# dsshim0125/s2p

Measured on AMD Instinct MI355X. Metric: G+D train-step images/sec at 84x84 bs=64/GPU, higher is better.
Workload: dtype bf16; 1 GPU; configs[2]: full G+D train step (hinge GAN + feature matching + VGG19 perceptual + L1, Adam x2), 84x84 cheetah, netG=s2p, netD=multiscale(2); global_batch=64, per_gpu_batch=64, parallelism=dp1, hip_graph=True, graph_segments=1, streams=overlapped, vgg_weights=seeded stand-in (ImageNet weights unobtainable offline)

## Files before the change

### include/s2p_hip.h

```cpp
#ifndef S2P_HIP_H
#define S2P_HIP_H
#include <stddef.h>
#include <stdint.h>

#ifdef __cplusplus
extern "C" {
#endif
#pragma GCC visibility push(default)

#define S2P_VERSION 125

enum { S2P_F32 = 0, S2P_BF16 = 1 };
enum { S2P_ACT_NONE = 0, S2P_ACT_RELU = 1, S2P_ACT_LRELU = 2, S2P_ACT_TANH = 3, S2P_ACT_SWISH = 4 };
enum { S2P_EPI_STORE = 0,
       S2P_EPI_ADD = 1,
       S2P_EPI_MUL_ACTGRAD = 2   };

typedef struct {
  int32_t dtype;
  int32_t N, H, W, Cin, x_pitch;
  int32_t Ho, Wo, Cout, y_pitch;
  int32_t KH, KW, stride, pad;
  int32_t transposed;
  int32_t reflect;
  int32_t groups;
  int32_t x_gstride, y_gstride;
  int32_t cin_real;
} s2p_conv_desc;

int s2p_version(void);
const char* s2p_last_error(void);

int s2p_conv2d_fwd(const s2p_conv_desc* d, const void* x, const void* w_fwd, const float* bias,
                   const void* aux, void* y, int act, float slope, int epi, void* stream);
int s2p_conv2d_dgrad(const s2p_conv_desc* d, const void* dy, const void* w_bwd,
                     const void* aux, const void* aux2, void* dx, int epi, int aux_act, float slope,
                     void* stream);
size_t s2p_conv2d_fwd_workspace(const s2p_conv_desc* d, int epi);
int s2p_conv2d_fwd_ws(const s2p_conv_desc* d, const void* x, const void* w_fwd, const float* bias,
                      const void* aux, void* y, int act, float slope, int epi, void* workspace,
                      size_t workspace_bytes, void* stream);
size_t s2p_conv2d_dgrad_workspace(const s2p_conv_desc* d);
int s2p_conv2d_dgrad_ws(const s2p_conv_desc* d, const void* dy, const void* w_bwd,
                        const void* aux, const void* aux2, void* dx, int epi, int aux_act, float slope,
                        void* workspace, size_t workspace_bytes, void* stream);
int s2p_conv2d_fwd_mat(const s2p_conv_desc* d, const void* x, const void* w_fwd, const float* bias, const void* aux,
                       void* y, int epi, const void* gb_img, int gb_pitch, const float* gb_st, int gb_st_pitch,
                       int act, float slope, float eps, void* y_mat, int y_mat_pitch, float* stats, void* workspace,
                       size_t workspace_bytes, void* stream);
int s2p_conv2d_dgrad_mat(const s2p_conv_desc* d, const void* dy, const void* w_bwd, void* d_mid, const void* aux, const void* xn,
                         int xn_pitch, const float* stats, const void* gb_img, int gb_pitch, const float* gb_st,
                         int gb_st_pitch, int act, float slope, float eps, float* sums, void* dxn, int dxn_pitch,
                         void* dgb_img, int dgb_pitch, float* dgb_st, int dgb_st_pitch, const void* res, int res_pitch,
                         void* workspace, size_t workspace_bytes, void* stream);
int s2p_conv2d_mat_is_fused(const s2p_conv_desc* d, int dgrad, int has_gb);
int s2p_conv2d_wgrad(const s2p_conv_desc* d, const void* x, const void* dy, float* dw, float* db,
                     int cin_real, int cout_real, int64_t dw_gstride, int splitk, void* stream);
size_t s2p_conv2d_wgrad_workspace(const s2p_conv_desc* d, int cin_real, int cout_real);
int s2p_conv2d_wgrad_ws(const s2p_conv_desc* d, const void* x, const void* dy, float* dw, float* db,
                        int cin_real, int cout_real, int64_t dw_gstride, int splitk, void* workspace,
                        size_t workspace_bytes, void* stream);
size_t s2p_conv2d_wgrad_det_workspace(const s2p_conv_desc* d, int cin_real, int cout_real, int splitk);
typedef struct { const void* x; const void* dy; float* dw; float* db; } s2p_wgrad_job;
size_t s2p_conv2d_wgrad_batched_workspace(const s2p_conv_desc* d, int n_jobs, int cin_real, int cout_real);
int s2p_conv2d_wgrad_batched(const s2p_conv_desc* d, const s2p_wgrad_job* jobs, int n_jobs, int cin_real,
                             int cout_real, void* workspace, size_t workspace_bytes, void* stream);
int s2p_reflect_pad_bwd(int dtype, const void* dxp, int N, int H, int W, int C, int pad, void* dx,
                        void* stream);
int s2p_channel_sum(int dtype, const void* dy, int64_t pixels, int C, int pitch, float* db,
                    void* stream);
size_t s2p_channel_sum_workspace(int64_t pixels, int C);
int s2p_channel_sum_ws(int dtype, const void* dy, int64_t pixels, int C, int pitch, float* db, void* workspace,
                       size_t workspace_bytes, void* stream);

int64_t s2p_in_stats_floats(int N, int HW, int C);
int s2p_in_stats(int dtype, const void* x, int N, int HW, int C, int pitch, float eps,
                 float* stats, void* stream);
int s2p_in_apply_fwd(int dtype, const void* x, int N, int HW, int C, int pitch,
                     const float* stats, const void* gb_img, int gb_pitch,
                     const float* gb_st, int gb_st_pitch, int act, float slope, float eps,
                     void* y, int y_pitch, void* stream);
int s2p_in_norm_fwd(int dtype, const void* x, int N, int HW, int C, int pitch, const void* gb_img, int gb_pitch,
                    const float* gb_st, int gb_st_pitch, int act, float slope, float eps, void* y, int y_pitch,
                    float* stats, void* stream);
int64_t s2p_in_bwd_sums_floats(int N, int HW, int C);
int s2p_in_bwd_reduce(int dtype, const void* da, int da_pitch, const void* x, int N, int HW, int C,
                      int pitch, const float* stats, const void* gb_img, int gb_pitch,
                      const float* gb_st, int gb_st_pitch, int act, float slope, float eps,
                      float* sums, void* stream);
int s2p_in_bwd_apply(int dtype, const void* da, int da_pitch, const void* x, int N, int HW, int C,
                     int pitch, const float* stats, const void* gb_img, int gb_pitch,
                     const float* gb_st, int gb_st_pitch, int act, float slope, float eps,
                     const float* sums, void* dx, int dx_pitch, void* dgb_img, int dgb_pitch,
                     float* dgb_st, int dgb_st_pitch, void* stream);

int s2p_posenc_fwd(const float* state, int N, int S, int L, float* out, int out_pitch, void* stream);

int s2p_in_norm_bwd(int dtype, const void* da, int da_pitch, const void* x, int N, int HW, int C, int pitch,
                    const float* stats, const void* gb_img, int gb_pitch, const float* gb_st, int gb_st_pitch,
                    int act, float slope, float eps, float* sums, void* dx, int dx_pitch, void* dgb_img,
                    int dgb_pitch, float* dgb_st, int dgb_st_pitch, void* stream);
int s2p_in_norm_bwd_res(int dtype, const void* da, int da_pitch, const void* x, int N, int HW, int C, int pitch,
                        const float* stats, const void* gb_img, int gb_pitch, const float* gb_st, int gb_st_pitch,
                        int act, float slope, float eps, float* sums, void* dx, int dx_pitch, void* dgb_img,
                        int dgb_pitch, float* dgb_st, int dgb_st_pitch, const void* res, int res_pitch, void* stream);

int s2p_linear_fwd(const float* x, int M, int K, int x_pitch, const float* w, int w_row, const float* bias, int N,
                   int act, float slope, float* y, int y_pitch, int n_store, void* stream);
size_t s2p_linear_bwd_workspace(int M, int K, int N);
int s2p_linear_bwd(const float* x, int x_pitch, const float* dy, int dy_pitch, const float* y, int y_pitch, int M,
                   int K, int k_real, int N, const float* w_bwd, int wb_row, int act, float slope, float* dw,
                   int dw_row, float* db, float* dx, int dx_pitch, void* workspace, size_t workspace_bytes,
                   void* stream);

int s2p_gauss_head_fwd(const float* raw, int raw_pitch, int M, int D, const float* eps, int eps_pitch, float* mean,
                       int mean_pitch, float* std, int std_pitch, float* z, int z_pitch, float* z2, int z2_pitch,
                       void* stream);
int s2p_gauss_head_bwd(const float* raw, int raw_pitch, int M, int D, const float* eps, int eps_pitch, const float* dmean,
                       int dmean_pitch, const float* dstd, int dstd_pitch, const float* dz, int dz_pitch, const float* dz2,
                       int dz2_pitch, float* draw, int draw_pitch, void* stream);
int s2p_linear_add_fwd(const float* x, int M, int K, int x_pitch, const float* w, int w_row, const float* bias, int N,
                       const float* add, int add_pitch, int act, float slope, float* y, int y_pitch, int n_store,
                       void* stream);
int s2p_linear_add_bwd(const float* x, int x_pitch, const float* dy, int dy_pitch, const float* y, int y_pitch, int M,
                       int K, int k_real, int N, const float* w_bwd, int wb_row, int act, float slope, float* dw,
                       int dw_row, float* db, float* dx, int dx_pitch, int dx_accumulate, float* dadd, int dadd_pitch,
                       void* stream);
int s2p_gauss_kl(const float* mu_p, const float* std_p, int p_pitch, const float* mu_q, const float* std_q, int q_pitch,
                 int B, int T, int D, int const_first, float scale, float* loss, float* dmu_p, float* dstd_p,
                 int dp_pitch, float* dmu_q, float* dstd_q, int dq_pitch, void* stream);
int s2p_gauss_ll(const float* mu, int mu_pitch, const float* std, int std_pitch, const float* target, const float* done,
                 int64_t n, float scale, float* loss, float* dmu, float* dstd, void* stream);
int s2p_gauss_ll_image(int dtype, const void* mu, int pitch, const void* target, int target_u8, int N, int C, int HW,
                       float sigma, float scale, float* loss, void* dmu, void* stream);

int s2p_avgpool3x3s2_fwd(int dtype, const void* x, int N, int H, int W, int C, void* y, void* stream);
int s2p_avgpool3x3s2_bwd(int dtype, const void* dy, int N, int H, int W, int C, void* dx,
                         int accumulate, void* stream);
int s2p_maxpool2x2_fwd(int dtype, const void* x, int N, int H, int W, int C, void* y, void* stream);
int s2p_maxpool2x2_bwd(int dtype, const void* dy, const void* x, int N, int H, int W, int C,
                       void* dx, void* stream);
int s2p_resize_nearest(int dtype, const void* x, int N, int H, int W, int C, void* y, int Ho, int Wo,
                       void* stream);
int s2p_nchw_to_nhwc(int dtype, const float* x, int N, int C, int H, int W, void* y, int y_pitch,
                     int c_off, int zero_pad, void* stream);
int s2p_nhwc_to_nchw(int dtype, const void* x, int x_pitch, int c_off, int N, int C, int H, int W,
                     float* y, int accumulate, void* stream);
int s2p_u8_to_nhwc(int dtype, const void* x, int64_t pixels, int C, void* y, int y_pitch, void* stream);
int s2p_nhwc_to_u8(int dtype, const void* x, int x_pitch, int64_t pixels, int C, void* y, void* stream);
int s2p_cast(int src_dtype, const void* src, int dst_dtype, void* dst, int64_t n, void* stream);

int s2p_l1_loss(int dtype, const void* a, const void* b, int64_t count, float scale,
                float* loss_out, void* grad_a, int accumulate, void* stream);
#define S2P_L1_MAX_JOBS 16
typedef struct { const void* a; const void* b; void* grad_a; int64_t count; float scale; float* loss_out; } s2p_l1_job;
int s2p_l1_loss_multi(int dtype, const s2p_l1_job* jobs, int n_jobs, void* stream);
int s2p_hinge_loss(int dtype, const void* x, int64_t count, int mode, float scale,
                   float* loss_out, void* grad_x, void* stream);
int s2p_hinge_loss_strided(int dtype, const void* x, int64_t pixels, int pitch, int mode, float scale,
                           float* loss_out, void* grad_x, void* stream);

int s2p_ensemble_head(const float* raw, int raw_pitch, const float* xin, int x_pitch, int B, int E, int D,
                      const float* min_logstd, const float* max_logstd, float* mean, float* std,
                      const int32_t* pick, const float* obs_mean, const float* obs_std, float rew_mean,
                      float rew_std, float* next_obs, float* reward, float* disagreement, float* aleatoric,
                      void* stream);

int s2p_ensemble_linear_fwd(const float* x, int64_t x_gstride, int x_pitch, const float* w, const float* bias,
                            const int32_t* member, int G, int E, int B, int K, int N, float* pre, float* act, int y_pitch,
                            void* stream);
int s2p_ensemble_linear_bwd(const float* x, int64_t x_gstride, int x_pitch, const float* dpre, int dpre_pitch,
                            const float* w, const int32_t* member, int G, int E, int B, int K, int N, float* dw, float* db,
                            const float* pre_prev, float* dprev, int prev_pitch, void* stream);
int s2p_ensemble_nll(const float* raw, int raw_pitch, const float* xin, int64_t x_gstride, int x_pitch, const float* target,
                     int64_t t_gstride, int t_pitch, int B, int G, int D, const float* min_logstd, const float* max_logstd,
                     float scale, float bound_reg, float* sums, float* loss, float* draw, int draw_pitch, float* dmin_logstd,
                     float* dmax_logstd, float* mean, float* std, void* stream);

int s2p_adam_step(float* p, const float* g, float* m, float* v, int64_t n, float lr, float beta1,
                  float beta2, float eps, int step, float grad_scale, void* stream);
int s2p_adam_step_dev(float* p, const float* g, float* m, float* v, int64_t n, float lr, float beta1,
                      float beta2, float eps, int* step_dev, float grad_scale, void* stream);
int s2p_adam_step_dev_part(float* p, const float* g, float* m, float* v, int64_t n, float lr, float beta1,
                           float beta2, float eps, int* step_dev, float grad_scale, int tick, void* stream);
typedef struct {
  const float* src; void* dst_fwd; void* dst_bwd;
  int32_t R, T, C;
  int32_t Cpad;
  int32_t Rrow;
  int32_t r_off;
  int32_t dtype;
} s2p_pack_job;
int s2p_pack_weights(const s2p_pack_job* jobs, int n_jobs, int max_elems, void* stream);
int s2p_pack_weights_scaled(const s2p_pack_job* jobs, const float* const* sigma, int n_jobs, int max_elems,
// ... 26 lines not shown
```

### s2p_amd/_lib.py

```python
import ctypes
import os
import subprocess

import torch

_HERE = os.path.dirname(os.path.abspath(__file__))
_SO = os.path.join(_HERE, "csrc", "libs2p_hip.so")

F32, BF16 = 0, 1
ACT_NONE, ACT_RELU, ACT_LRELU, ACT_TANH, ACT_SWISH = 0, 1, 2, 3, 4
EPI_STORE, EPI_ADD, EPI_MUL_ACTGRAD = 0, 1, 2

c_int, c_float, c_void_p, c_int64 = ctypes.c_int, ctypes.c_float, ctypes.c_void_p, ctypes.c_int64


class ConvDesc(ctypes.Structure):
    _fields_ = [(n, ctypes.c_int32) for n in (
        "dtype", "N", "H", "W", "Cin", "x_pitch", "Ho", "Wo", "Cout", "y_pitch",
        "KH", "KW", "stride", "pad", "transposed", "reflect", "groups", "x_gstride", "y_gstride", "cin_real")]


class L1Job(ctypes.Structure):
    _fields_ = [("a", c_void_p), ("b", c_void_p), ("grad_a", c_void_p), ("count", c_int64), ("scale", c_float),
                ("loss_out", c_void_p)]


class WgradJob(ctypes.Structure):
    _fields_ = [("x", c_void_p), ("dy", c_void_p), ("dw", c_void_p), ("db", c_void_p)]


class PackJob(ctypes.Structure):
    _fields_ = [("src", c_void_p), ("dst_fwd", c_void_p), ("dst_bwd", c_void_p),
                ("R", ctypes.c_int32), ("T", ctypes.c_int32), ("C", ctypes.c_int32),
                ("Cpad", ctypes.c_int32), ("Rrow", ctypes.c_int32), ("r_off", ctypes.c_int32),
                ("dtype", ctypes.c_int32)]


class SnJob(ctypes.Structure):
    _fields_ = [("w", c_void_p), ("u", c_void_p), ("v", c_void_p), ("sigma", c_void_p), ("ws", c_void_p), ("grad", c_void_p),
                ("R", ctypes.c_int32), ("K", ctypes.c_int32)]


_P = c_void_p
_DESC = ctypes.POINTER(ConvDesc)
SIGNATURES = {
    "s2p_version": [],
    "s2p_last_error": [],
    "s2p_conv2d_fwd": [_DESC, _P, _P, _P, _P, _P, c_int, c_float, c_int, _P],
    "s2p_conv2d_dgrad": [_DESC, _P, _P, _P, _P, _P, c_int, c_int, c_float, _P],
    "s2p_conv2d_fwd_workspace": [_DESC, c_int],
    "s2p_conv2d_fwd_ws": [_DESC, _P, _P, _P, _P, _P, c_int, c_float, c_int, _P, ctypes.c_size_t, _P],
    "s2p_conv2d_fwd_mat": [_DESC, _P, _P, _P, _P, _P, c_int, _P, c_int, _P, c_int, c_int, c_float, c_float, _P, c_int, _P, _P,
                           ctypes.c_size_t, _P],
    "s2p_conv2d_dgrad_mat": [_DESC, _P, _P, _P, _P, _P, c_int, _P, _P, c_int, _P, c_int, c_int, c_float, c_float, _P, _P, c_int, _P, c_int,
                             _P, c_int, _P, c_int, _P, ctypes.c_size_t, _P],
    "s2p_conv2d_mat_is_fused": [_DESC, c_int, c_int],
    "s2p_conv2d_dgrad_workspace": [_DESC],
    "s2p_conv2d_dgrad_ws": [_DESC, _P, _P, _P, _P, _P, c_int, c_int, c_float, _P, ctypes.c_size_t, _P],
    "s2p_conv2d_wgrad": [_DESC, _P, _P, _P, _P, c_int, c_int, c_int64, c_int, _P],
    "s2p_conv2d_wgrad_workspace": [_DESC, c_int, c_int],
    "s2p_conv2d_wgrad_det_workspace": [_DESC, c_int, c_int, c_int],
    "s2p_channel_sum_workspace": [c_int64, c_int],
    "s2p_channel_sum_ws": [c_int, _P, c_int64, c_int, c_int, _P, _P, ctypes.c_size_t, _P],
    "s2p_conv2d_wgrad_ws": [_DESC, _P, _P, _P, _P, c_int, c_int, c_int64, c_int, _P, ctypes.c_size_t, _P],
    "s2p_conv2d_wgrad_batched_workspace": [_DESC, c_int, c_int, c_int],
    "s2p_conv2d_wgrad_batched": [_DESC, ctypes.POINTER(WgradJob), c_int, c_int, c_int, _P, ctypes.c_size_t, _P],
    "s2p_reflect_pad_bwd": [c_int, _P, c_int, c_int, c_int, c_int, c_int, _P, _P],
    "s2p_channel_sum": [c_int, _P, c_int64, c_int, c_int, _P, _P],
    "s2p_in_stats": [c_int, _P, c_int, c_int, c_int, c_int, c_float, _P, _P],
    "s2p_in_apply_fwd": [c_int, _P, c_int, c_int, c_int, c_int, _P, _P, c_int, _P, c_int, c_int, c_float,
                         c_float, _P, c_int, _P],
    "s2p_in_norm_fwd": [c_int, _P, c_int, c_int, c_int, c_int, _P, c_int, _P, c_int, c_int, c_float, c_float, _P, c_int,
                        _P, _P],
    "s2p_in_bwd_reduce": [c_int, _P, c_int, _P, c_int, c_int, c_int, c_int, _P, _P, c_int, _P, c_int, c_int,
                          c_float, c_float, _P, _P],
    "s2p_in_bwd_apply": [c_int, _P, c_int, _P, c_int, c_int, c_int, c_int, _P, _P, c_int, _P, c_int, c_int,
                         c_float, c_float, _P, _P, c_int, _P, c_int, _P, c_int, _P],
    "s2p_in_norm_bwd": [c_int, _P, c_int, _P, c_int, c_int, c_int, c_int, _P, _P, c_int, _P, c_int, c_int,
                        c_float, c_float, _P, _P, c_int, _P, c_int, _P, c_int, _P],
    "s2p_in_norm_bwd_res": [c_int, _P, c_int, _P, c_int, c_int, c_int, c_int, _P, _P, c_int, _P, c_int, c_int,
                            c_float, c_float, _P, _P, c_int, _P, c_int, _P, c_int, _P, c_int, _P],
    "s2p_in_stats_floats": [c_int, c_int, c_int],
    "s2p_in_bwd_sums_floats": [c_int, c_int, c_int],
    "s2p_linear_fwd": [_P, c_int, c_int, c_int, _P, c_int, _P, c_int, c_int, c_float, _P, c_int, c_int, _P],
    "s2p_linear_bwd_workspace": [c_int, c_int, c_int],
    "s2p_linear_bwd": [_P, c_int, _P, c_int, _P, c_int, c_int, c_int, c_int, c_int, _P, c_int, c_int, c_float, _P, c_int, _P, _P,
                       c_int, _P, ctypes.c_size_t, _P],
    "s2p_gauss_head_fwd": [_P, c_int, c_int, c_int, _P, c_int, _P, c_int, _P, c_int, _P, c_int, _P, c_int, _P],
    "s2p_gauss_head_bwd": [_P, c_int, c_int, c_int, _P, c_int, _P, c_int, _P, c_int, _P, c_int, _P, c_int, _P, c_int, _P],
    "s2p_linear_add_fwd": [_P, c_int, c_int, c_int, _P, c_int, _P, c_int, _P, c_int, c_int, c_float, _P, c_int, c_int, _P],
    "s2p_linear_add_bwd": [_P, c_int, _P, c_int, _P, c_int, c_int, c_int, c_int, c_int, _P, c_int, c_int, c_float, _P, c_int, _P, _P,
                           c_int, c_int, _P, c_int, _P],
    "s2p_gauss_kl": [_P, _P, c_int, _P, _P, c_int, c_int, c_int, c_int, c_int, c_float, _P, _P, _P, c_int, _P, _P, c_int, _P],
    "s2p_gauss_ll": [_P, c_int, _P, c_int, _P, _P, c_int64, c_float, _P, _P, _P, _P],
    "s2p_gauss_ll_image": [c_int, _P, c_int, _P, c_int, c_int, c_int, c_int, c_float, c_float, _P, _P, _P],
    "s2p_posenc_fwd": [_P, c_int, c_int, c_int, _P, c_int, _P],
    "s2p_avgpool3x3s2_fwd": [c_int, _P, c_int, c_int, c_int, c_int, _P, _P],
    "s2p_avgpool3x3s2_bwd": [c_int, _P, c_int, c_int, c_int, c_int, _P, c_int, _P],
    "s2p_maxpool2x2_fwd": [c_int, _P, c_int, c_int, c_int, c_int, _P, _P],
    "s2p_maxpool2x2_bwd": [c_int, _P, _P, c_int, c_int, c_int, c_int, _P, _P],
    "s2p_resize_nearest": [c_int, _P, c_int, c_int, c_int, c_int, _P, c_int, c_int, _P],
    "s2p_nchw_to_nhwc": [c_int, _P, c_int, c_int, c_int, c_int, _P, c_int, c_int, c_int, _P],
    "s2p_nhwc_to_nchw": [c_int, _P, c_int, c_int, c_int, c_int, c_int, c_int, _P, c_int, _P],
    "s2p_cast": [c_int, _P, c_int, _P, c_int64, _P],
    "s2p_u8_to_nhwc": [c_int, _P, c_int64, c_int, _P, c_int, _P],
    "s2p_nhwc_to_u8": [c_int, _P, c_int, c_int64, c_int, _P, _P],
    "s2p_l1_loss": [c_int, _P, _P, c_int64, c_float, _P, _P, c_int, _P],
    "s2p_l1_loss_multi": [c_int, ctypes.POINTER(L1Job), c_int, _P],
    "s2p_hinge_loss": [c_int, _P, c_int64, c_int, c_float, _P, _P, _P],
    "s2p_hinge_loss_strided": [c_int, _P, c_int64, c_int, c_int, c_float, _P, _P, _P],
    "s2p_adam_step": [_P, _P, _P, _P, c_int64, c_float, c_float, c_float, c_float, c_int, c_float, _P],
    "s2p_ensemble_head": [_P, c_int, _P, c_int, c_int, c_int, c_int, _P, _P, _P, _P, _P, _P, _P, c_float, c_float, _P, _P,
                          _P, _P, _P],
    "s2p_ensemble_linear_fwd": [_P, c_int64, c_int, _P, _P, ctypes.POINTER(ctypes.c_int32), c_int, c_int, c_int, c_int, c_int, _P, _P,
                                c_int, _P],
    "s2p_ensemble_linear_bwd": [_P, c_int64, c_int, _P, c_int, _P, ctypes.POINTER(ctypes.c_int32), c_int, c_int, c_int, c_int, c_int,
                                _P, _P, _P, _P, c_int, _P],
    "s2p_ensemble_nll": [_P, c_int, _P, c_int64, c_int, _P, c_int64, c_int, c_int, c_int, c_int, _P, _P, c_float, c_float,
                         _P, _P, _P, c_int, _P, _P, _P, _P, _P],
    "s2p_adam_step_dev": [_P, _P, _P, _P, c_int64, c_float, c_float, c_float, c_float, _P, c_float, _P],
    "s2p_adam_step_dev_part": [_P, _P, _P, _P, c_int64, c_float, c_float, c_float, c_float, _P, c_float, c_int, _P],
    "s2p_pack_weights": [_P, c_int, c_int, _P],
    "s2p_pack_weights_scaled": [_P, _P, c_int, c_int, _P],
    "s2p_sn_workspace_floats": [c_int, c_int],
    "s2p_sn_power_iter": [_P, c_int, c_int, c_int, c_int, _P],
    "s2p_sn_project_grad": [_P, c_int, c_int, c_int, _P],
    "s2p_act_bwd": [c_int, _P, _P, c_int64, c_int, c_float, _P, _P],
    "s2p_scale": [c_int, _P, c_int64, _P, _P],
    "s2p_add": [c_int, _P, _P, _P, c_int64, _P],
    "s2p_copy_channels": [c_int, _P, c_int, c_int, _P, c_int, c_int, c_int, c_int64, c_int, _P],
    "s2p_image_metrics": [_P, _P, c_int, c_int, c_int, c_int, c_float, _P, _P, _P],
}
_RESTYPE = {"s2p_last_error": ctypes.c_char_p, "s2p_conv2d_wgrad_det_workspace": ctypes.c_size_t, "s2p_channel_sum_workspace": ctypes.c_size_t, "s2p_conv2d_wgrad_batched_workspace": ctypes.c_size_t, "s2p_conv2d_wgrad_workspace": ctypes.c_size_t, "s2p_conv2d_fwd_workspace": ctypes.c_size_t, "s2p_conv2d_dgrad_workspace": ctypes.c_size_t, "s2p_linear_bwd_workspace": ctypes.c_size_t, "s2p_in_stats_floats": c_int64, "s2p_in_bwd_sums_floats": c_int64,
            "s2p_sn_workspace_floats": c_int64}

_lib = None


def build(force=False):
    script = os.path.join(_HERE, "csrc", "build.sh")
    env = dict(os.environ)
    if force:
        env["FORCE"] = "1"
    subprocess.check_call(["bash", script], env=env)
    return os.path.join(_HERE, "csrc", "libs2p_hip.so")


def lib():
    global _lib
    if _lib is None:
        if not os.path.exists(_SO):
            raise RuntimeError(
                f"libs2p_hip.so not found at {_SO}: the S2P hot path has no CPU fallback; run "
# ... 41 lines not shown
```

### s2p_amd/csrc/conv_igemm.hip

```cpp
#include "s2p_common.h"
#include "conv_plane.h"
#include "conv_planeg.h"
#include <type_traits>
#include <vector>

#define MAX_TAPS 64

constexpr int PHASE_TAPS = 16, MAX_PHASES = 4;
struct GatherArgs {
  const void* x; const void* w; const float* bias; const void* aux; const void* aux2; void* y;
  int M, Hi, Wi, Qh, Qw;
  int Cin, x_pitch, x_gstride;
  int Cout, Cst, y_pitch, y_gstride;
  int Ho, Wo;
  int istride, ostride, oy0, ox0;
  int T, Ktot, w_row;
  long long w_gstride;
  int reflect, act, epi, gact;
  float slope, gslope;
  int npix_tiles, nco_tiles;
  int halo_lo, halo_hi;
  int diag;
  int splitk, ksteps;
  float* part; int psplit, psteps, part_m;
// ... 1113 lines not shown
      prow[j] = ok ? hb + hp * RS : zrow;
      psw[j] = ok ? (hp >> 1) & 7 : 0;
    }
    if (S2P_DIAGV(a) != 2) {
      bf16x8 af[4][TCO], bf[4][TPIX];
#pragma unroll
      for (int s = 0; s < 4; ++s) {
#pragma unroll
        for (int i = 0; i < TCO; ++i) af[s][i] = *(const bf16x8*)(wrow + i * 32 * RS + (((2 * s + h) ^ swr) * 16));
#pragma unroll
        for (int j = 0; j < TPIX; ++j) bf[s][j] = *(const bf16x8*)(prow[j] + (((2 * s + h) ^ psw[j]) * 16));
      }
      __builtin_amdgcn_sched_barrier(0);
#pragma unroll
      for (int s = 0; s < 4; ++s)
#pragma unroll
        for (int i = 0; i < TCO; ++i)
#pragma unroll
          for (int j = 0; j < TPIX; ++j)
            acc[i][j] = __builtin_amdgcn_mfma_f32_32x32x16_bf16(af[s][i], bf[s][j], acc[i][j], 0, 0, 0);
    }
    __syncthreads();
    tap = ntap;
    tw_cur = tw_next; tw_next = tw_next2;
    if (nslab_i != slab) {
      slab = nslab_i;
      if (!DBUF && slab < nslab) {
        issue_halo(0, slab * BK);
        __syncthreads();
      }
    }
  }
  (void)nk;
  if (S2P_DIAGV(a) == 8) {
    const unsigned long long c1 = __builtin_amdgcn_s_memtime(), r1 = __builtin_amdgcn_s_memrealtime();
    if (tid == 0 && g == 0) {
      unsigned long long* o = (unsigned long long*)a.y + (size_t)blockIdx.x * 2;
      o[0] = c1 - st_c0; o[1] = r1 - st_r0;
    }
    if (acc[0][0][0] == 12345.678f) ((float*)a.y)[7] = acc[1][1][3] + acc[0][1][2] + acc[1][0][1];
    return;
  }
  if (S2P_DIAGV(a) == 4) { if (acc[0][0][0] == 12345.678f) ((float*)a.y)[0] = acc[1][1][3] + acc[0][1][2] + acc[1][0][1]; return; }
  conv_epilogue<T, BCO, BPIX, TCO, TPIX>(a, acc, smem, rowoff, g, co_base, wco0, wpix0, r, h, tid);
}

enum class ConvPath { Thin, Thin4, ThinCin, ThinRows, Plane, PlaneG, Halo, SplitK, Dma, Fast, Phases, Generic };
enum class HaloKind { S9_176_PIPE, S9_176, S9_320, R_176, R_320 };

struct ConvOperands {
  const void* x; const void* w; const float* bias; const void* aux; const void* aux2; void* y;
  int act; float slope; int epi, gact; float gslope;
};
struct NormWant { bool any, gb, bwd; };
struct ScratchAvail { bool any; size_t bytes; };
static const ScratchAvail SCRATCH_UNLIMITED{true, ~(size_t)0};
struct Scratch { void* ws; size_t bytes; };

struct GatherChoice {
  ConvPath path = ConvPath::Generic;
  bool fused = false;
  size_t ws_bytes = 0;
  int bco = 128;
  HaloKind halo = HaloKind::R_320;
  PlaneArgs plane;
  PlaneGArgs planeg;
};
struct GatherItem { GatherArgs a; GatherChoice c; };
struct ConvPlan {
  ConvPath path = ConvPath::Generic;
  bool fused = false;
  size_t ws_bytes = 0;
  int cout_pad = 0;
  std::vector<GatherItem> items;
  void add(const GatherItem& it) {
    if (items.empty()) path = it.c.path;
    if (it.c.ws_bytes > ws_bytes) ws_bytes = it.c.ws_bytes;
    items.push_back(it);
    fused = items.size() == 1 && it.c.fused;
  }
};

template <typename P>
static void copy_conv_fields(P& p, const GatherArgs& a) {
  p.x = a.x; p.w = a.w; p.bias = a.bias; p.aux = a.aux; p.aux2 = a.aux2; p.y = a.y;
  p.Cin = a.Cin; p.x_pitch = a.x_pitch; p.x_gstride = a.x_gstride;
  p.Cout = a.Cout; p.Cst = a.Cst; p.y_pitch = a.y_pitch; p.y_gstride = a.y_gstride;
  p.w_row = a.w_row; p.w_gstride = a.w_gstride;
  p.act = a.act; p.epi = a.epi; p.gact = a.gact; p.slope = a.slope; p.gslope = a.gslope;
  p.x_bytes = a.x_bytes; p.w_bytes = a.w_bytes;
}
template <typename P>
static void copy_norm(P& p, const PlaneMat& m) {
  p.xn = m.xn; p.xn_pitch = m.xn_pitch; p.dgb = m.dgb; p.dgb_pitch = m.dgb_pitch;
  p.dgbst = m.dgbst; p.dgbst_pitch = m.dgbst_pitch; p.res = m.res; p.res_pitch = m.res_pitch;
  p.y2 = m.y2; p.y2_pitch = m.y2_pitch; p.gb = m.gb; p.gb_pitch = m.gb_pitch;
  p.gbst = m.gbst; p.gbst_pitch = m.gbst_pitch; p.stats = m.stats;
  p.n_act = m.act; p.n_slope = m.slope; p.eps = m.eps;
}

static void plan_fast(GatherArgs& a, GatherChoice& c, int groups, const NormWant& want, const ScratchAvail& sc) {
  const ConvSwitches& sw = conv_switches();
  a.npix_tiles = cdiv(a.M, 128);
  a.nco_tiles = cdiv(a.Cst, c.bco);
  a.diag = sw.diag;
  const int nwg = a.npix_tiles * a.nco_tiles;
  const bool whole = a.ostride == 1 && a.oy0 == 0 && a.ox0 == 0 && a.Qh == a.Ho && a.Qw == a.Wo;
  const bool planes = whole && a.M % (a.Qh * a.Qw) == 0;
  int S = 1;
  if (!sw.no_dma && !sw.no_split && groups == 1 && whole && sc.any) S = conv_split_plan(nwg, a.Ktot / 64);
  if (!sw.no_plane && !sw.no_dma && a.T == 9 && a.istride == 1 && planes && a.Qh == a.Hi && a.Qw == a.Wi) {
    PlaneArgs& p = c.plane;
    bool ok = true;
    for (int t = 0; t < 9; ++t) p.wt[t] = -1;
    for (int t = 0; t < 9 && ok; ++t) {
      const int dy = (int)(signed char)(a.tap[t] & 0xff), dx = (int)(signed char)((a.tap[t] >> 8) & 0xff);
      if (dy < -1 || dy > 1 || dx < -1 || dx > 1 || p.wt[(dy + 1) * 3 + dx + 1] >= 0) ok = false;
      else p.wt[(dy + 1) * 3 + dx + 1] = a.tap[t] >> 16;
    }
    copy_conv_fields(p, a);
    p.N = a.M / (a.Qh * a.Qw); p.H = a.Qh; p.W = a.Qw;
    if (ok && s2p_conv_plane_applicable(p)) {
      c.path = ConvPath::Plane;
      c.fused = want.any && groups == 1 && a.act == S2P_ACT_NONE && a.epi != S2P_EPI_MUL_ACTGRAD && (!want.bwd || a.epi == S2P_EPI_STORE);
      return;
    }
  }
  if (!sw.no_plane && !sw.no_planeg() && !(a.T == 9 && sw.no_planeg_3x3()) && !sw.no_dma && groups == 1 && planes && !a.reflect) {
    PlaneGProblem pr{a.M / (a.Qh * a.Qw), a.Hi, a.Wi, a.Ho, a.Wo, a.Cin, a.Cout, a.Cst, a.x_pitch, a.y_pitch, a.istride, a.T, a.tap, want.any};
    PlaneGArgs& p = c.planeg;
    if (s2p_conv_planeg_setup(pr, p)) {
      copy_conv_fields(p, a);
      p.N = pr.N;
      c.path = ConvPath::PlaneG;
      c.fused = want.any && p.nbands == 1 && p.gimg == 1 && !want.gb && a.act == S2P_ACT_NONE && a.epi != S2P_EPI_MUL_ACTGRAD;
      return;
    }
  }
  if (c.bco == 128 && S <= 1 && !sw.no_dma && !sw.no_halo && a.istride == 1 && a.ostride == 1 && a.Qh == a.Hi && a.Qw == a.Wi &&
      a.Ho == a.Qh && a.Wo == a.Qw && a.T >= 4) {
    int lo = 0, hi = 0;
    for (int t = 0; t < a.T; ++t) {
      int off = (int)(signed char)(a.tap[t] & 0xff) * a.Wi + (int)(signed char)((a.tap[t] >> 8) & 0xff);
      if (-off > lo) lo = -off;
      if (off > hi) hi = off;
    }
    const int npos = 128 + lo + hi;
    const bool s9 = a.T == 9 && !sw.no_static_taps;
    if (npos <= 320) {
      a.halo_lo = lo; a.halo_hi = hi;
      c.path = ConvPath::Halo;
      if (npos <= 176) c.halo = s9 ? (sw.halo_pipe && a.Cin % 64 == 0 ? HaloKind::S9_176_PIPE : HaloKind::S9_176) : HaloKind::R_176;
      else c.halo = s9 ? HaloKind::S9_320 : HaloKind::R_320;
      return;
    }
  }
  if (S > 1) {
    const int nk = a.Ktot / 64;
    a.psteps = cdiv(nk, S); a.psplit = cdiv(nk, a.psteps);
    a.part_m = a.npix_tiles * 128;
    const size_t need = (size_t)a.psplit * a.Cst * a.part_m * sizeof(float);
    if (a.psplit > 1 && need <= sc.bytes) { c.path = ConvPath::SplitK; c.ws_bytes = need; return; }
    a.psplit = 1;
  }
  c.path = sw.no_dma ? ConvPath::Fast : ConvPath::Dma;
}

static GatherItem plan_gather(const GatherArgs& a_in, bool bf16, int groups, long long x_elems, const NormWant& want, const ScratchAvail& sc) {
  GatherItem it{a_in, {}};
  GatherArgs& a = it.a;
  const long long xb = x_elems * 2, wb = (long long)a.Cout * a.w_row * 2;
  if (bf16 && a.Cin % 64 == 0 && !a.reflect && a.T > 0 && xb < (1ll << 31) && wb < (1ll << 31) && a.Cst > 32) {
    a.x_bytes = (unsigned)xb; a.w_bytes = (unsigned)wb;
    it.c.bco = a.Cst > 64 ? 128 : 64;
    plan_fast(a, it.c, groups, want, sc);
  }
  return it;
}

static int pack_tap(int dy, int dx, int wt) { return (wt << 16) | ((dx & 0xff) << 8) | (dy & 0xff); }

struct Geo {
  int N, Hi, Wi, Ci, xp, xg, Ho, Wo, Co, Cst, yp, yg, KH, KW, stride, pad, reflect, groups;
  long long w_gstride; int w_row;
};

static inline long long gathered_elems(const Geo& G) {
  const long long one = (long long)G.N * G.Hi * G.Wi * G.xp;
// ... 138 lines not shown
  if (d->reflect) { H += 2 * pad; W += 2 * pad; pad = 0; }
  Geo G{d->N, d->Ho, d->Wo, cout_pad, d->y_pitch, d->y_gstride, H, W, d->Cin, d->Cin,
        d->x_pitch, d->x_gstride, d->KH, d->KW, d->stride, pad, 0, d->groups,
        (long long)d->Cin * d->KH * d->KW * cout_pad, d->KH * d->KW * cout_pad};
  if (d->transposed) return plan_gather_problem(G, d->dtype == S2P_BF16, op, want, sc, P);
  return plan_scatter_problem(G, d->dtype == S2P_BF16, op, want, sc, P);
}

template <int BCO>
static int launch_bf16(GatherArgs& a, const GatherChoice& c, int groups, void* ws, hipStream_t st) {
  const int extra_lds = conv_switches().halo_extra_lds;
  dim3 grid(a.npix_tiles * a.nco_tiles, groups);
  switch (c.path) {
    case ConvPath::Halo:
      if constexpr (BCO == 128) {
        switch (c.halo) {
          case HaloKind::S9_176_PIPE: hipLaunchKernelGGL((conv_halo_kernel<176, true, 9, true>), grid, dim3(256), extra_lds, st, a); break;
          case HaloKind::S9_176: hipLaunchKernelGGL((conv_halo_kernel<176, true, 9>), grid, dim3(256), extra_lds, st, a); break;
          case HaloKind::S9_320: hipLaunchKernelGGL((conv_halo_kernel<320, false, 9>), grid, dim3(256), 0, st, a); break;
          case HaloKind::R_176: hipLaunchKernelGGL((conv_halo_kernel<176, true>), grid, dim3(256), extra_lds, st, a); break;
          case HaloKind::R_320: hipLaunchKernelGGL((conv_halo_kernel<320, false>), grid, dim3(256), 0, st, a); break;
        }
        S2P_CHECK_LAUNCH("conv_halo_kernel");
      }
      return 0;
    case ConvPath::SplitK: {
      a.part = (float*)ws;
      grid.z = a.psplit;
      hipLaunchKernelGGL((conv_dma_kernel<BCO, 128, 2, 2>), grid, dim3(256), 0, st, a);
      S2P_CHECK_LAUNCH("conv_dma_kernel(split)");
      const long long n = (long long)(a.part_m / 4) * ((a.Cst + 7) / 8);
      hipLaunchKernelGGL(conv_part_reduce_kernel, dim3(cdiv(n, 64)), dim3(64), 0, st, a);
      S2P_CHECK_LAUNCH("conv_part_reduce_kernel");
      return 0;
    }
    case ConvPath::Fast:
      hipLaunchKernelGGL((conv_fast_kernel<BCO, 128, 2, 2>), grid, dim3(256), 0, st, a);
      S2P_CHECK_LAUNCH("conv_fast_kernel");
      return 0;
    default:
      hipLaunchKernelGGL((conv_dma_kernel<BCO, 128, 2, 2>), grid, dim3(256), 0, st, a);
      S2P_CHECK_LAUNCH("conv_dma_kernel");
      return 0;
  }
}

template <typename T>
static int launch_generic(GatherArgs& a, int groups, hipStream_t st) {
  if (a.Cst > 64) return launch_cfg<T, 128, 128, 2, 2>(a, groups, st);
  if (a.Cst > 32) return launch_cfg<T, 64, 128, 2, 2>(a, groups, st);
  return launch_cfg<T, 32, 256, 1, 4>(a, groups, st);
}

static int launch_item(GatherItem& it, bool bf16, int groups, const PlaneMat* mat, void* ws, hipStream_t st) {
  if (!bf16) return launch_generic<float>(it.a, groups, st);
  switch (it.c.path) {
    case ConvPath::Plane:
      if (it.c.fused) copy_norm(it.c.plane, *mat);
      return s2p_conv_plane_launch(it.c.plane, groups, st);
    case ConvPath::PlaneG:
      if (it.c.fused) copy_norm(it.c.planeg, *mat);
      return s2p_conv_planeg_launch(it.c.planeg, groups, st);
    case ConvPath::Phases: {
      GatherArgs& a = it.a;
      int max_npt = 0;
      for (int i = 0; i < a.nphase; ++i) if (a.ph[i].npix_tiles > max_npt) max_npt = a.ph[i].npix_tiles;
      const dim3 grid = a.phase_fast ? dim3(((max_npt * a.nco_tiles + 7) / 8) * 8 * a.nphase, groups, 1) : dim3(max_npt * a.nco_tiles, groups, a.nphase);
      if (it.c.bco == 128) hipLaunchKernelGGL((conv_dma_kernel<128, 128, 2, 2>), grid, dim3(256), 0, st, a);
      else hipLaunchKernelGGL((conv_dma_kernel<64, 128, 2, 2>), grid, dim3(256), 0, st, a);
      S2P_CHECK_LAUNCH("conv_dma_kernel(phases)");
      return 0;
    }
    case ConvPath::Generic: break;
    default: return it.c.bco == 128 ? launch_bf16<128>(it.a, it.c, groups, ws, st) : launch_bf16<64>(it.a, it.c, groups, ws, st);
  }
  return launch_generic<__bf16>(it.a, groups, st);
}
static int launch_items(ConvPlan& P, bool bf16, int groups, const PlaneMat* mat, const Scratch& sc, hipStream_t st) {
  for (GatherItem& it : P.items) {
    const int rc = launch_item(it, bf16, groups, mat, sc.ws, st);
    if (rc) return rc;
  }
  return 0;
}

static int conv_fwd_impl(const s2p_conv_desc* d, const ConvOperands& op, const PlaneMat* mat, bool* fused, const Scratch& sc, void* stream) {
  S2P_CHECK_SLOPE("s2p_conv2d_fwd", op.act, op.slope);
  if (mat) S2P_CHECK_SLOPE("s2p_conv2d_fwd_mat", mat->act, mat->slope);
  ConvPlan P;
  int rc = conv_plan_fwd(d, op, NormWant{mat != nullptr, mat && mat->gb, false}, ScratchAvail{sc.ws != nullptr, sc.bytes}, P);
  if (rc) return rc;
  if (!op.x || !op.w || (!op.y && !mat)) S2P_FAIL(-1, "s2p_conv2d_fwd: null pointer");
  if (op.epi != S2P_EPI_STORE && !op.aux) S2P_FAIL(-1, "s2p_conv2d_fwd: epi needs aux");
  if (!op.y && !P.fused) S2P_FAIL(-1, "s2p_conv2d_fwd_mat: y == NULL needs the fused launch (s2p_conv2d_mat_is_fused)");
  if (fused) *fused = P.fused;
  hipStream_t st = (hipStream_t)stream;
  switch (P.path) {
    case ConvPath::Thin: return s2p_thin_fwd(d, op.x, op.w, op.bias, op.y, op.act, op.slope, st);
    case ConvPath::Thin4: return s2p_thin4_fwd(d, op.x, op.w, op.bias, op.y, op.act, op.slope, sc.ws, sc.bytes, st);
    case ConvPath::ThinCin: return s2p_thin_cin_fwd(d, op.x, op.w, op.bias, op.y, op.act, op.slope, st);
    default: return launch_items(P, d->dtype == S2P_BF16, d->groups, mat, sc, st);
  }
}

extern "C" int s2p_conv2d_fwd(const s2p_conv_desc* d, const void* x, const void* w_fwd, const float* bias,
                              const void* aux, void* y, int act, float slope, int epi, void* stream) {
  return conv_fwd_impl(d, ConvOperands{x, w_fwd, bias, aux, nullptr, y, act, slope, epi, 0, 0.f}, nullptr, nullptr, Scratch{nullptr, 0}, stream);
}
extern "C" int s2p_conv2d_fwd_ws(const s2p_conv_desc* d, const void* x, const void* w_fwd, const float* bias,
                                 const void* aux, void* y, int act, float slope, int epi, void* workspace,
                                 size_t workspace_bytes, void* stream) {
  return conv_fwd_impl(d, ConvOperands{x, w_fwd, bias, aux, nullptr, y, act, slope, epi, 0, 0.f}, nullptr, nullptr,
                       Scratch{workspace, workspace_bytes}, stream);
}
extern "C" int s2p_conv2d_fwd_mat(const s2p_conv_desc* d, const void* x, const void* w_fwd, const float* bias, const void* aux,
                                  void* y, int epi, const void* gb_img, int gb_pitch, const float* gb_st, int gb_st_pitch,
                                  int act, float slope, float eps, void* y_mat, int y_mat_pitch, float* stats, void* workspace,
                                  size_t workspace_bytes, void* stream) {
  if (!d || !y_mat || !stats) S2P_FAIL(-1, "s2p_conv2d_fwd_mat: null pointer");
  if (act != S2P_ACT_NONE && act != S2P_ACT_RELU && act != S2P_ACT_LRELU) S2P_FAIL(-1, "s2p_conv2d_fwd_mat: activation must be none / relu / lrelu");
  if (d->groups != 1 || d->transposed) S2P_FAIL(-1, "s2p_conv2d_fwd_mat: groups == 1, not transposed");
  PlaneMat m{y_mat, y_mat_pitch, gb_img, gb_pitch, gb_st, gb_st_pitch, stats, act, slope, eps, nullptr, 0, nullptr, 0, nullptr, 0, nullptr, 0};
  bool fused = false;
  int rc = conv_fwd_impl(d, ConvOperands{x, w_fwd, bias, aux, nullptr, y, S2P_ACT_NONE, 0.f, epi, 0, 0.f}, &m, &fused,
                         Scratch{workspace, workspace_bytes}, stream);
  if (rc || fused) return rc;
  return s2p_in_norm_fwd(d->dtype, y, d->N, d->Ho * d->Wo, d->Cout, d->y_pitch, gb_img, gb_pitch, gb_st, gb_st_pitch, act, slope,
                         eps, y_mat, y_mat_pitch, stats, stream);
}
extern "C" size_t s2p_conv2d_fwd_workspace(const s2p_conv_desc* d, int epi) {
  ConvPlan P;
  if (conv_plan_fwd(d, ConvOperands{nullptr, nullptr, nullptr, nullptr, nullptr, nullptr, S2P_ACT_NONE, 0.f, epi, 0, 0.f}, NormWant{}, SCRATCH_UNLIMITED, P)) return 0;
  return P.ws_bytes;
}

static int conv_dgrad_impl(const s2p_conv_desc* d, const ConvOperands& op, const PlaneMat* mat, bool must_fuse, bool* fused, const Scratch& sc,
                           void* stream) {
  if (op.epi == S2P_EPI_MUL_ACTGRAD) S2P_CHECK_ACT_FROM_OUT("s2p_conv2d_dgrad (aux_act)", op.gact);
  ConvPlan P;
  int rc = conv_plan_dgrad(d, op, NormWant{mat != nullptr, mat && mat->gb, true}, ScratchAvail{sc.ws != nullptr, sc.bytes}, P);
  if (rc) return rc;
  if (!op.x || !op.w || !op.y) S2P_FAIL(-1, "s2p_conv2d_dgrad: null pointer");
  if (op.epi != S2P_EPI_STORE && !op.aux) S2P_FAIL(-1, "s2p_conv2d_dgrad: epi needs aux");
  if (must_fuse && !P.fused)
    S2P_FAIL(-1, "s2p_conv2d_dgrad_mat: dgrad and norm backward are two launches for these arguments (s2p_conv2d_mat_is_fused; an aux "
                 "gradient fuses only on the 4x4 family): d_mid and sums are required");
  if (fused) *fused = P.fused;
  hipStream_t st = (hipStream_t)stream;
  switch (P.path) {
    case ConvPath::Thin4: return s2p_thin4_dgrad(d, op.x, op.w, op.y, P.cout_pad, sc.ws, sc.bytes, st);
    case ConvPath::ThinRows: return s2p_thin_rows_dgrad(d, op.x, op.w, op.y, P.cout_pad, st);
    default: return launch_items(P, d->dtype == S2P_BF16, d->groups, mat, sc, st);
  }
}

extern "C" int s2p_conv2d_dgrad(const s2p_conv_desc* d, const void* dy, const void* w_bwd, const void* aux,
                                const void* aux2, void* dx, int epi, int aux_act, float slope, void* stream) {
  return conv_dgrad_impl(d, ConvOperands{dy, w_bwd, nullptr, aux, aux2, dx, S2P_ACT_NONE, 0.f, epi, aux_act, slope}, nullptr, false, nullptr,
                         Scratch{nullptr, 0}, stream);
}
extern "C" int s2p_conv2d_dgrad_ws(const s2p_conv_desc* d, const void* dy, const void* w_bwd, const void* aux,
                                   const void* aux2, void* dx, int epi, int aux_act, float slope, void* workspace,
                                   size_t workspace_bytes, void* stream) {
  return conv_dgrad_impl(d, ConvOperands{dy, w_bwd, nullptr, aux, aux2, dx, S2P_ACT_NONE, 0.f, epi, aux_act, slope}, nullptr, false, nullptr,
                         Scratch{workspace, workspace_bytes}, stream);
}
extern "C" int s2p_conv2d_dgrad_mat(const s2p_conv_desc* d, const void* dy, const void* w_bwd, void* d_mid, const void* aux, const void* xn,
                                    int xn_pitch, const float* stats, const void* gb_img, int gb_pitch, const float* gb_st,
                                    int gb_st_pitch, int act, float slope, float eps, float* sums, void* dxn, int dxn_pitch,
                                    void* dgb_img, int dgb_pitch, float* dgb_st, int dgb_st_pitch, const void* res, int res_pitch,
                                    void* workspace, size_t workspace_bytes, void* stream) {
  if (!d || !xn || !stats || !dxn) S2P_FAIL(-1, "s2p_conv2d_dgrad_mat: null pointer");
  if (act != S2P_ACT_NONE && act != S2P_ACT_RELU && act != S2P_ACT_LRELU) S2P_FAIL(-1, "s2p_conv2d_dgrad_mat: activation must be none / relu / lrelu");
  if (d->groups != 1 || d->transposed || d->reflect) S2P_FAIL(-1, "s2p_conv2d_dgrad_mat: groups == 1, not transposed, zero padding");
  if (d->Cin != d->x_pitch) S2P_FAIL(-1, "s2p_conv2d_dgrad_mat: the produced tensor must be dense (x_pitch %d != Cin %d)", d->x_pitch, d->Cin);
  PlaneMat m{dxn, dxn_pitch, gb_img, gb_pitch, gb_st, gb_st_pitch, const_cast<float*>(stats), act, slope, eps,
             xn, xn_pitch, dgb_img, dgb_pitch, dgb_st, dgb_st_pitch, res, res_pitch};
  bool fused = false;
  int rc = conv_dgrad_impl(d, ConvOperands{dy, w_bwd, nullptr, aux, nullptr, d_mid ? d_mid : dxn, S2P_ACT_NONE, 0.f,
                                           aux ? S2P_EPI_ADD : S2P_EPI_STORE, S2P_ACT_NONE, 0.f},
                           &m, !d_mid || !sums, &fused, Scratch{workspace, workspace_bytes}, stream);
  if (rc || fused) return rc;
  return s2p_in_norm_bwd_res(d->dtype, d_mid, d->x_pitch, xn, d->N, d->H * d->W, d->Cin, xn_pitch, stats, gb_img, gb_pitch, gb_st,
                             gb_st_pitch, act, slope, eps, sums, dxn, dxn_pitch, dgb_img, dgb_pitch, dgb_st, dgb_st_pitch, res,
                             res_pitch, stream);
}
extern "C" int s2p_conv2d_mat_is_fused(const s2p_conv_desc* d, int dgrad, int has_gb) {
  if (!d || d->groups != 1 || d->transposed || d->reflect) return 0;
  const ConvOperands op{nullptr, nullptr, nullptr, nullptr, nullptr, nullptr, S2P_ACT_NONE, 0.f, S2P_EPI_STORE, S2P_ACT_NONE, 0.f};
  const NormWant want{true, has_gb != 0, dgrad != 0};
  ConvPlan P;
  const int rc = dgrad ? conv_plan_dgrad(d, op, want, SCRATCH_UNLIMITED, P) : conv_plan_fwd(d, op, want, SCRATCH_UNLIMITED, P);
  return rc == 0 && P.fused ? 1 : 0;
}
extern "C" size_t s2p_conv2d_dgrad_workspace(const s2p_conv_desc* d) {
  ConvPlan P;
  if (conv_plan_dgrad(d, ConvOperands{nullptr, nullptr, nullptr, nullptr, nullptr, nullptr, S2P_ACT_NONE, 0.f, S2P_EPI_STORE, S2P_ACT_NONE, 0.f},
                      NormWant{}, SCRATCH_UNLIMITED, P)) return 0;
  return P.ws_bytes;
}
```

### s2p_amd/csrc/conv_plane.h

```cpp
#pragma once
#include <hip/hip_runtime.h>

struct PlaneMat {
  void* y2; int y2_pitch; const void* gb; int gb_pitch; const float* gbst; int gbst_pitch; float* stats; int act; float slope, eps;
  const void* xn; int xn_pitch; void* dgb; int dgb_pitch; float* dgbst; int dgbst_pitch; const void* res; int res_pitch;
};

struct PlaneArgs {
  const void* x; const void* w; const float* bias; const void* aux; const void* aux2; void* y;
  int N, H, W;
  int Cin, x_pitch, x_gstride;
  int Cout, Cst, y_pitch, y_gstride;
  int w_row;
  long long w_gstride;
  int wt[9];
  int act, epi, gact;
  float slope, gslope;
  unsigned x_bytes, w_bytes;
  void* y2; int y2_pitch;
  const void* gb; int gb_pitch;
  const float* gbst; int gbst_pitch;
  float* stats; int n_act; float n_slope, eps;
  const void* xn; int xn_pitch; void* dgb; int dgb_pitch; float* dgbst; int dgbst_pitch; const void* res; int res_pitch;
  int nco, gxcd;
  int diag;
};

bool s2p_conv_plane_applicable(const PlaneArgs& a);
int s2p_conv_plane_launch(PlaneArgs& a, int groups, hipStream_t st);
```

### s2p_amd/csrc/conv_plane.hip

```cpp
#include "s2p_common.h"
#include "conv_plane.h"
#include <type_traits>

typedef __attribute__((ext_vector_type(4))) float f32x4v;

__device__ __forceinline__ void pl_dma16(i32x4 rsrc, unsigned lds_dst, int voffset, int soffset) {
  asm volatile("s_mov_b32 m0, %2\n\ts_nop 0\n\tbuffer_load_dwordx4 %0, %1, %3 offen lds"
               :: "v"(voffset), "s"(rsrc), "s"(lds_dst), "s"(soffset) : "memory", "m0");
}

namespace {
constexpr int PL_NPOS = 512;
constexpr int PL_CPS = PL_NPOS * 32;
constexpr int PL_PBUF = 2 * PL_CPS;
constexpr int PL_WST = 4096;
constexpr int PL_RING = 6;
constexpr int PL_ERS = 144;
}

template <int PB, int WP, int DIAG, int MAT = 0, int GST = 0>
__global__ __launch_bounds__(512) void conv_plane_kernel(const PlaneArgs a) {
  typedef __bf16 T;
  static_assert(GST == 0 || (MAT != 0 && DIAG == 0 && PB == 7), "gamma|beta staging: fused-norm product kernels only");
  constexpr int BPIX = 4 * PB * 16;
  constexpr int NT = 4 * PB;
  constexpr int MERGE = 4 * NT * 1024;
  constexpr int MAIN = 2 * PL_PBUF + PL_RING * PL_WST;
  constexpr int EPI = BPIX * PL_ERS;
  constexpr int SMEM = GST ? 163840 : (MERGE > MAIN ? (MERGE > EPI ? MERGE : EPI) : (MAIN > EPI ? MAIN : EPI));
  constexpr int XOFF = GST ? PL_PBUF : 0;
  constexpr int GB_B = MAIN;
  constexpr int GB_ROWS_B = (163840 - MAIN) / 256, GB_ROWS = GB_ROWS_B + 96;
  static_assert(!GST || (GB_ROWS_B == 288 && BPIX * 128 == MAIN - PL_PBUF), "LDS map of the staged form");
  __shared__ __attribute__((aligned(1024))) char smem[SMEM];
  char* const pbase = smem;
  char* const wbase = smem + 2 * PL_PBUF;

  unsigned long long ph[6] = {0, 0, 0, 0, 0, 0};
  if constexpr ((DIAG & 128) != 0) ph[0] = __builtin_amdgcn_s_memrealtime();
  const int tid = threadIdx.x;
  const int lane = tid & 63;
  const int wave = __builtin_amdgcn_readfirstlane(tid >> 6);
  const int set = wave >> 2, wq = wave & 3;
  const int q = lane >> 4, l15 = lane & 15;
  const int g = blockIdx.y;
  int img, cs;
  {
    const int bid = blockIdx.x, nco = a.nco;
    if ((a.N & 7) == 0) { const int xcd = bid & 7, k = bid >> 3; cs = k % nco; img = (k / nco) * 8 + xcd; }
    else { cs = bid % nco; img = bid / nco; }
  }
  const int co_base = cs * 64;
  const int HW = a.H * a.W;

  const T* xg = (const T*)a.x + (size_t)g * a.x_gstride;
  const T* wg = (const T*)a.w + (size_t)g * a.w_gstride;
  const i32x4 xrs = s2p_make_rsrc(xg, a.x_bytes - (unsigned)g * (unsigned)a.x_gstride * 2u);
  const i32x4 wrs = s2p_make_rsrc(wg, a.w_bytes);
  const unsigned p_lds = __builtin_amdgcn_readfirstlane(s2p_lds_addr(pbase));
  const unsigned w_lds = __builtin_amdgcn_readfirstlane(s2p_lds_addr(wbase));
  const unsigned OOB = 0x80000000u;

  int hv[4]; unsigned hdst[4];
#pragma unroll
  for (int k = 0; k < 4; ++k) {
    const int ii = wave + 8 * k;
    const int cp = ii & 1, pg = ii >> 1;
    const int pos = 32 * pg + (lane >> 1);
    const int pm = pos - 1;
    const int yy = pm / WP - 1, xx = pm % WP;
    const bool ok = pos >= 1 && yy >= 0 && yy < a.H && xx < a.W;
    hv[k] = ok ? (int)((((unsigned)(img * a.H + yy) * a.W + xx) * a.x_pitch) * 2u + (2 * cp + (lane & 1)) * 16) : (int)OOB;
    hdst[k] = (unsigned)(cp * PL_CPS + pg * 1024);
    if constexpr ((DIAG & 64) != 0) hv[k] = (int)(((unsigned)img * a.H * a.W * a.x_pitch) * 2u + ii * 1024 + lane * 16);
  }
// ... 274 lines not shown
    float bv[2][4];
#pragma unroll
    for (int i = 0; i < 2; ++i)
#pragma unroll
      for (int e = 0; e < 4; ++e) bv[i][e] = bias ? bias[16 * (IB + i) + 4 * q + e] : 0.f;
    auto stage_out = [&](auto f) {
#pragma unroll
      for (int i = 0; i < 2; ++i)
#pragma unroll
        for (int j = 0; j < PB; ++j) {
          const int px = (wq * PB + j) * 16 + l15;
          const f32x4v v = acc[IB + i][j];
          bf16x4 o = {(__bf16)f(v[0] + bv[i][0]), (__bf16)f(v[1] + bv[i][1]), (__bf16)f(v[2] + bv[i][2]), (__bf16)f(v[3] + bv[i][3])};
          *(bf16x4*)(srow(px, 2 * (IB + i) + (q >> 1)) + (q & 1) * 8) = o;
        }
    };
    if (a.act == S2P_ACT_TANH) stage_out([](float v) { return tanhf(v); });
    else if (a.act == S2P_ACT_SWISH) stage_out([](float v) { return v / (1.f + expf(-v)); });
    else if (a.act == S2P_ACT_NONE) stage_out([](float v) { return v; });
    else {
      const float ns = a.act == S2P_ACT_RELU ? 0.f : a.slope;
      stage_out([ns](float v) { return lrelu_ns(v, ns); });
    }
  };
  if (set == 0) finish(std::integral_constant<int, 0>{}); else finish(std::integral_constant<int, 2>{});
  __syncthreads();
  if constexpr ((DIAG & 128) != 0) ph[4] = __builtin_amdgcn_s_memrealtime();
  T* yg = (T*)a.y + (size_t)g * a.y_gstride;
  const T* auxg = a.aux ? (const T*)a.aux + (size_t)g * a.y_gstride : nullptr;
  const T* aux2g = a.aux2 ? (const T*)a.aux2 + (size_t)g * a.y_gstride : nullptr;
  const bool epi_add = a.epi == S2P_EPI_ADD;
  const bool g_tanh = a.gact == S2P_ACT_TANH;
  const float gneg = a.gact == S2P_ACT_RELU ? 0.f : (a.gact == S2P_ACT_LRELU ? a.gslope : 1.f);
  auto out_chunk = [&](int row, int ch, size_t go, const Chunk<T>* pre = nullptr) {
    Chunk<T> c;
    c.raw = *(const u32x4*)srow(row, ch);
    if (a.epi != S2P_EPI_STORE) {
      Chunk<T> x, x2;
      if (pre) x = *pre; else x.raw = *(const u32x4*)(auxg + go);
      x2.raw = (u32x4){0u, 0u, 0u, 0u};
      if (aux2g) x2.raw = *(const u32x4*)(aux2g + go);
      float ov[8];
#pragma unroll
      for (int e = 0; e < 8; ++e) {
        float v = c.get(e), xv = x.get(e);
        const float f = g_tanh ? 1.f - xv * xv : (xv > 0.f ? 1.f : gneg);
        ov[e] = epi_add ? v + xv : (v + x2.get(e)) * f;
      }
      c.pack(ov);
    }
    return c;
  };
  if constexpr (MAT == 0) {
    for (int idx = tid; idx < HW * 8; idx += 512) {
      const int row = idx >> 3, ch = idx & 7;
      const size_t go = ((size_t)img * HW + row) * a.y_pitch + co_base + ch * 8;
      *(u32x4*)(yg + go) = out_chunk(row, ch, go).raw;
    }
  } else if constexpr (MAT == 1) {
    constexpr int MAXR = BPIX / 64;
    const int ch = tid & 7, r0 = tid >> 3;
    const T* gbb = a.gb ? (const T*)a.gb + (size_t)img * HW * a.gb_pitch + co_base + ch * 8 : nullptr;
    constexpr int KG0 = GST ? GB_ROWS / 64 : 0;
    static_assert(!GST || KG0 == T_KG0, "row groups staged in LDS");
    Chunk<T> xv[MAXR], gv[MAXR - KG0], bv[MAXR - KG0];
#pragma unroll
    for (int k = KG0; k < MAXR; ++k) {
      const int row = r0 + 64 * k;
      if constexpr (GST != 0) { gv[k - KG0] = pre_g[k - KG0]; bv[k - KG0] = pre_b[k - KG0]; }
      else {
        gv[k - KG0].raw = (u32x4){0u, 0u, 0u, 0u}; bv[k - KG0].raw = gv[k - KG0].raw;
        if (gbb && row < HW) {
          gv[k - KG0].raw = *(const u32x4*)(gbb + (size_t)row * a.gb_pitch);
          bv[k - KG0].raw = *(const u32x4*)(gbb + (size_t)row * a.gb_pitch + a.Cout);
        }
      }
    }
    auto gst_row = [&](int k) -> int {
      const int row = r0 + 64 * k;
      return (row < GB_ROWS_B ? GB_B + row * 256 : (row - GB_ROWS_B) * 256) + ((r0 & 1) << 7) + ch * 16;
    };
    float xf[MAXR][8];
#pragma unroll
    for (int k = 0; k < MAXR; ++k) {
      const int row = r0 + 64 * k;
      xv[k].raw = (u32x4){0u, 0u, 0u, 0u};
      if (row < HW) {
        const size_t go = ((size_t)img * HW + row) * a.y_pitch + co_base + ch * 8;
        if constexpr (GST != 0) xv[k] = out_chunk(row, ch, go, &pre_a[k]); else xv[k] = out_chunk(row, ch, go);
        if (a.y) *(u32x4*)(yg + go) = xv[k].raw;
      }
      xv[k].unpack(xf[k]);
    }
    __syncthreads();
    float* red = (float*)(smem + XOFF);
    float* cst = red + 8 * 64;
    auto plane_sum = [&](float (&v)[8], int slot) {
#pragma unroll
      for (int e = 0; e < 8; ++e) {
#pragma unroll
        for (int o = 8; o < 64; o <<= 1) v[e] += __shfl_xor(v[e], o, 64);
      }
      __syncthreads();
      if (lane < 8) {
#pragma unroll
        for (int e = 0; e < 8; ++e) red[wave * 64 + lane * 8 + e] = v[e];
      }
      __syncthreads();
      if (tid < 64) {
        float t = 0.f;
// ... 157 lines not shown
      if (a.dgbst) {
        a.dgbst[(size_t)img * a.dgbst_pitch + c] = t2;
        a.dgbst[(size_t)img * a.dgbst_pitch + a.Cout + c] = t3;
      }
    }
    __syncthreads();
    T* dxo = (T*)a.y2 + (size_t)img * HW * a.y2_pitch + lc;
    T* dgo = a.dgb ? (T*)a.dgb + (size_t)img * HW * a.dgb_pitch + lc : nullptr;
    const T* rsb = a.res ? (const T*)a.res + (size_t)img * HW * a.res_pitch + lc : nullptr;
    float rr2[8], g12[8], s1v[8], s2v[8];
#pragma unroll
    for (int e = 0; e < 8; ++e) { const int cl = ch * 8 + e; rr2[e] = cst[64 + cl]; g12[e] = cst[128 + cl]; s1v[e] = cst[256 + cl]; s2v[e] = cst[320 + cl]; }
#pragma unroll
    for (int k = 0; k < MAXR; ++k) {
      const int row = r0 + 64 * k;
      if (row >= HW) break;
      Chunk<T> o0, o1, o2, gk, bk;
      load_gb(k, gk, bk);
      float v0[8], v1[8];
#pragma unroll
      for (int e = 0; e < 8; ++e) {
        const float gg = g12[e] + gk.get(e);
        const float xh = xhf[k][e], dy = dyf[k][e];
        const float dxh = dy * gg;
        v0[e] = rr2[e] * (dxh - s1v[e] - xh * s2v[e]);
        v1[e] = dy * xh;
      }
      if (rsb) {
        Chunk<T> rv; rv.raw = *(const u32x4*)(rsb + (size_t)row * a.res_pitch);
        o0.pack(v0);
#pragma unroll
        for (int e = 0; e < 8; ++e) v0[e] = o0.get(e) + rv.get(e);
      }
      o0.pack(v0); o1.pack(v1); o2.pack(dyf[k]);
      *(u32x4*)(dxo + (size_t)row * a.y2_pitch) = o0.raw;
      if (dgo) {
        *(u32x4*)(dgo + (size_t)row * a.dgb_pitch) = o1.raw;
        *(u32x4*)(dgo + (size_t)row * a.dgb_pitch + a.Cout) = o2.raw;
      }
    }
  }
  if constexpr ((DIAG & 128) != 0) {
    asm volatile("s_waitcnt vmcnt(0)" ::: "memory");
    __syncthreads();
    ph[5] = __builtin_amdgcn_s_memrealtime();
    if (tid == 0 && g == 0 && a.aux && a.epi == S2P_EPI_STORE) {
      unsigned long long* o = (unsigned long long*)a.aux + (size_t)blockIdx.x * 8;
#pragma unroll
      for (int k = 0; k < 6; ++k) o[k] = ph[k];
    }
  }
}

template <int PB, int WP, int DIAG>
__global__ __launch_bounds__(512) void conv_plane_pair_kernel(const PlaneArgs a) {
  typedef __bf16 T;
  constexpr int BPIX = 4 * PB * 16;
  constexpr int RINGB = PL_RING * PL_WST;
  constexpr int MAIN = 2 * PL_PBUF + 2 * RINGB;
  constexpr int EPI = BPIX * PL_ERS;
  constexpr int SMEM = 2 * EPI > MAIN ? 2 * EPI : MAIN;
  __shared__ __attribute__((aligned(1024))) char smem[SMEM];
  char* const pbase = smem;
  const int tid = threadIdx.x;
  const int lane = tid & 63;
  const int wave = __builtin_amdgcn_readfirstlane(tid >> 6);
  const int set = wave >> 2, wq = wave & 3;
  const int q = lane >> 4, l15 = lane & 15;
  int g = blockIdx.y;
  int img, cpair;
  {
    const int bid = blockIdx.x, np = a.nco >> 1;
    if (a.gxcd) {
      const int L = blockIdx.y * gridDim.x + bid, xcd = L & 7, j = L >> 3;
      const int per_unit = (a.N >> 1) * np;
      const int u = xcd + 8 * (j / per_unit), r = j % per_unit;
      g = u >> 1; cpair = r % np; img = (u & 1) * (a.N >> 1) + r / np;
    } else if ((a.N & 7) == 0) { const int xcd = bid & 7, k = bid >> 3; cpair = k % np; img = (k / np) * 8 + xcd; }
    else { cpair = bid % np; img = bid / np; }
  }
  const int co_base = (2 * cpair + set) * 64;
  const int HW = a.H * a.W;
  char* const wbase = smem + 2 * PL_PBUF + set * RINGB;
  const T* xg = (const T*)a.x + (size_t)g * a.x_gstride;
  const T* wg = (const T*)a.w + (size_t)g * a.w_gstride;
  const i32x4 xrs = s2p_make_rsrc(xg, a.x_bytes - (unsigned)g * (unsigned)a.x_gstride * 2u);
  const i32x4 wrs = s2p_make_rsrc(wg, a.w_bytes);
  const unsigned p_lds = __builtin_amdgcn_readfirstlane(s2p_lds_addr(pbase));
  const unsigned w_lds = __builtin_amdgcn_readfirstlane(s2p_lds_addr(wbase));
  const unsigned OOB = 0x80000000u;
  int hv[4]; unsigned hdst[4];
#pragma unroll
  for (int k = 0; k < 4; ++k) {
    const int ii = wave + 8 * k;
    const int cp = ii & 1, pg = ii >> 1;
    const int pos = 32 * pg + (lane >> 1);
    const int pm = pos - 1;
    const int yy = pm / WP - 1, xx = pm % WP;
    const bool ok = pos >= 1 && yy >= 0 && yy < a.H && xx < a.W;
    hv[k] = ok ? (int)((((unsigned)(img * a.H + yy) * a.W + xx) * a.x_pitch) * 2u + (2 * cp + (lane & 1)) * 16) : (int)OOB;
    hdst[k] = (unsigned)(cp * PL_CPS + pg * 1024);
  }
  int wv; unsigned wdst;
  {
    const int cp = wave & 1, cohalf = (wave >> 1) & 1;
    const int co = co_base + 32 * cohalf + (lane >> 1);
    wv = co < a.Cout ? (int)((unsigned)co * a.w_row * 2u + (2 * cp + (lane & 1)) * 16) : (int)OOB;
// ... 83 lines not shown
      __builtin_amdgcn_sched_barrier(0);
      read_b(un{}, I4{}, nb); read_b(un{}, I5{}, nb);
      mfma4(I4{}, fa, fb);
      __builtin_amdgcn_sched_barrier(0);
      read_b(un{}, I6{}, nb);
      mfma4(I5{}, fa, fb);
      __builtin_amdgcn_sched_barrier(0);
      mfma4(I6{}, fa, fb);
      __builtin_amdgcn_sched_barrier(0);
#pragma unroll
      for (int i = 0; i < 4; ++i) fa[i] = na[i];
#pragma unroll
      for (int j = 0; j < PB; ++j) fb[j] = nb[j];
    });
  }
  S2P_WAIT_VMCNT(0);
  asm volatile("s_waitcnt lgkmcnt(0)" ::: "memory");
  __syncthreads();
  {
    char* stg = smem + set * EPI;
    const float* bias = a.bias ? a.bias + (size_t)g * a.Cout + co_base : nullptr;
    float bv[4][4];
#pragma unroll
    for (int i = 0; i < 4; ++i)
#pragma unroll
      for (int e = 0; e < 4; ++e) bv[i][e] = bias ? bias[16 * i + 4 * q + e] : 0.f;
    auto stage_out = [&](auto f) {
#pragma unroll
      for (int i = 0; i < 4; ++i)
#pragma unroll
        for (int j = 0; j < PB; ++j) {
          const int px = (wq * PB + j) * 16 + l15;
          const f32x4v v = acc[i][j];
          bf16x4 o = {(__bf16)f(v[0] + bv[i][0]), (__bf16)f(v[1] + bv[i][1]), (__bf16)f(v[2] + bv[i][2]), (__bf16)f(v[3] + bv[i][3])};
          *(bf16x4*)(stg + px * PL_ERS + (16 * i + 4 * q) * 2) = o;
        }
    };
    if (a.act == S2P_ACT_TANH) stage_out([](float v) { return tanhf(v); });
    else if (a.act == S2P_ACT_SWISH) stage_out([](float v) { return v / (1.f + expf(-v)); });
    else if (a.act == S2P_ACT_NONE) stage_out([](float v) { return v; });
    else {
      const float ns = a.act == S2P_ACT_RELU ? 0.f : a.slope;
      stage_out([ns](float v) { return lrelu_ns(v, ns); });
    }
  }
  __syncthreads();
  {
    T* yg = (T*)a.y + (size_t)g * a.y_gstride;
    const T* auxg = a.aux ? (const T*)a.aux + (size_t)g * a.y_gstride : nullptr;
    const T* aux2g = a.aux2 ? (const T*)a.aux2 + (size_t)g * a.y_gstride : nullptr;
    const bool epi_add = a.epi == S2P_EPI_ADD;
    const bool g_tanh = a.gact == S2P_ACT_TANH;
    const float gneg = a.gact == S2P_ACT_RELU ? 0.f : (a.gact == S2P_ACT_LRELU ? a.gslope : 1.f);
    for (int idx = tid; idx < HW * 16; idx += 512) {
      const int row = idx >> 4, ch16 = idx & 15, sl = ch16 >> 3, ch = ch16 & 7;
      Chunk<T> c;
      c.raw = *(const u32x4*)(smem + sl * EPI + row * PL_ERS + ch * 16);
      const size_t go = ((size_t)img * HW + row) * a.y_pitch + (2 * cpair + sl) * 64 + ch * 8;
      if (a.epi != S2P_EPI_STORE) {
        Chunk<T> x, x2;
        x.raw = *(const u32x4*)(auxg + go);
        x2.raw = (u32x4){0u, 0u, 0u, 0u};
        if (aux2g) x2.raw = *(const u32x4*)(aux2g + go);
        float ov[8];
#pragma unroll
        for (int e = 0; e < 8; ++e) {
          float v = c.get(e), xv = x.get(e);
          const float f = g_tanh ? 1.f - xv * xv : (xv > 0.f ? 1.f : gneg);
          ov[e] = epi_add ? v + xv : (v + x2.get(e)) * f;
        }
        c.pack(ov);
      }
      *(u32x4*)(yg + go) = c.raw;
    }
  }
}

bool s2p_conv_plane_applicable(const PlaneArgs& a) {
  if (a.H > 21 || a.W > 21 || a.H < 3 || a.W < 3) return false;
  const int HW = a.H * a.W;
  if (HW > 448 || HW <= 320) return false;
  if (a.Cin % 64 || a.Cout % 64 || a.Cst != a.Cout) return false;
  if (a.y_pitch % 8 || a.x_pitch % 8) return false;
  return true;
}

int s2p_conv_plane_launch(PlaneArgs& a, int groups, hipStream_t st) {
  a.nco = a.Cout / 64;
  dim3 grid(a.N * a.nco, groups);
#ifdef S2P_DIAG_BUILD
  static const int diag = s2p_env_int("S2P_DIAG", 0);
#define PL_DIAG_CASE(D) if (diag == D) { hipLaunchKernelGGL((conv_plane_kernel<7, 22, D>), grid, dim3(512), 0, st, a); S2P_CHECK_LAUNCH("conv_plane_kernel(diag)"); return 0; }
  PL_DIAG_CASE(1) PL_DIAG_CASE(2) PL_DIAG_CASE(4) PL_DIAG_CASE(5) PL_DIAG_CASE(8) PL_DIAG_CASE(16) PL_DIAG_CASE(17) PL_DIAG_CASE(20) PL_DIAG_CASE(21) PL_DIAG_CASE(64) PL_DIAG_CASE(128)
#undef PL_DIAG_CASE
#endif
  if (!a.y2 && (a.nco & 1) == 0 && (long long)a.N * a.nco * groups > 256 && !s2p_env_set("S2P_NO_PLANE_PAIR")) {
    dim3 gp(a.N * (a.nco / 2), groups);
    a.gxcd = (groups > 1 && (2 * groups) % 8 == 0 && a.N % 2 == 0 && gp.x % 8 == 0 && !S2P_DIAG_SWITCH(17)) ? 1 : 0;
    hipLaunchKernelGGL((conv_plane_pair_kernel<7, 22, 0>), gp, dim3(512), 0, st, a);
    S2P_CHECK_LAUNCH("conv_plane_pair_kernel");
    return 0;
  }
  const bool gst = a.y2 && a.gb && a.Cin >= 256 && a.H * a.W >= 384 && (long long)a.N * a.H * a.W * a.gb_pitch * 2 < (1ll << 31) && !S2P_DIAG_SWITCH(7);
  if (a.y2 && a.xn) {
    if (gst) hipLaunchKernelGGL((conv_plane_kernel<7, 22, 0, 2, 1>), grid, dim3(512), 0, st, a);
    else hipLaunchKernelGGL((conv_plane_kernel<7, 22, 0, 2>), grid, dim3(512), 0, st, a);
    S2P_CHECK_LAUNCH("conv_plane_kernel(mat bwd)"); return 0;
  }
  if (a.y2) {
    if (gst) hipLaunchKernelGGL((conv_plane_kernel<7, 22, 0, 1, 1>), grid, dim3(512), 0, st, a);
    else hipLaunchKernelGGL((conv_plane_kernel<7, 22, 0, 1>), grid, dim3(512), 0, st, a);
    S2P_CHECK_LAUNCH("conv_plane_kernel(mat)"); return 0;
  }
  hipLaunchKernelGGL((conv_plane_kernel<7, 22, 0>), grid, dim3(512), 0, st, a);
  S2P_CHECK_LAUNCH("conv_plane_kernel");
  return 0;
}
```

### s2p_amd/csrc/conv_planeg.h

```cpp
#pragma once
#include <hip/hip_runtime.h>

struct PlaneGArgs {
  const void* x; const void* w; const float* bias; const void* aux; const void* aux2; void* y;
  int N;
  int H, W;
  int Ho, Wo;
  int WP, PT, PL;
  int Hs, Ws;
  int Cin, x_pitch, x_gstride;
  int Cout, Cst, y_pitch, y_gstride;
  int w_row;
  long long w_gstride;
  int wt[16];
  int act, epi, gact;
  float slope, gslope;
  unsigned x_bytes, w_bytes;
  void* y2; int y2_pitch;
  const void* gb; int gb_pitch;
  const float* gbst; int gbst_pitch;
  float* stats; int n_act; float n_slope, eps;
  const void* xn; int xn_pitch; void* dgb; int dgb_pitch; float* dgbst; int dgbst_pitch; const void* res; int res_pitch;
  int nco, img_xcd;
  int R, nbands;
  int shape;
  int gimg, Hst;
};

struct PlaneGProblem {
  int N, Hi, Wi, Ho, Wo, Cin, Cout, Cst, x_pitch, y_pitch, istride, T;
  const int* tap;
  bool want_mat;
};
bool s2p_conv_planeg_setup(const PlaneGProblem& p, PlaneGArgs& a);
int s2p_conv_planeg_launch(PlaneGArgs& a, int groups, hipStream_t st);
```

### s2p_amd/csrc/conv_planeg.hip

```cpp
#include "s2p_common.h"
#include "conv_planeg.h"
#include <type_traits>

typedef __attribute__((ext_vector_type(4))) float f32x4v;

__device__ __forceinline__ void pg_dma16(i32x4 rsrc, unsigned lds_dst, int voffset, int soffset) {
  asm volatile("s_mov_b32 m0, %2\n\ts_nop 0\n\tbuffer_load_dwordx4 %0, %1, %3 offen lds"
               :: "v"(voffset), "s"(rsrc), "s"(lds_dst), "s"(soffset) : "memory", "m0");
}

#ifndef PG_OCC4_ALL
#define PG_OCC4_ALL 0
#endif
namespace {
constexpr int PG_WST = 4096;
constexpr int PG_ERS = 144;

template <int T, int PPW> struct PgSched {
  static constexpr bool EARLY1 = T >= 6;
  static constexpr int W1_END = EARLY1 ? (T - 2) / 2 - 2 : -1;
  static constexpr int W0_BEG = (T - 3) / 2 + 1, W0_END = T - 3;
  static constexpr int PER1 = EARLY1 ? (PPW + W1_END) / (W1_END + 1) : PPW;
  static constexpr int PER0 = EARLY1 ? (PPW + (W0_END - W0_BEG)) / (W0_END - W0_BEG + 1) : PPW;
  static constexpr int Q1 = PER1 < 2 ? 2 : PER1, Q0 = PER0 < 2 ? 2 : PER0;
// ... 237 lines not shown
    const float* bias = a.bias ? a.bias + (size_t)g * a.Cout + co_base : nullptr;
    float bv[2][4];
#pragma unroll
    for (int i = 0; i < 2; ++i)
#pragma unroll
      for (int e = 0; e < 4; ++e) bv[i][e] = bias ? bias[16 * (IB + i) + 4 * q + e] : 0.f;
    auto stage_out = [&](auto f) {
#pragma unroll
      for (int i = 0; i < 2; ++i)
#pragma unroll
        for (int j = 0; j < PB; ++j) {
          const int px = (wq * PB + j) * 16 + l15;
          const f32x4v v = acc[IB + i][j];
          bf16x4 o = {(__bf16)f(v[0] + bv[i][0]), (__bf16)f(v[1] + bv[i][1]), (__bf16)f(v[2] + bv[i][2]), (__bf16)f(v[3] + bv[i][3])};
          *(bf16x4*)(smem + px * PG_ERS + (16 * (IB + i) + 4 * q) * 2) = o;
        }
    };
    if (a.act == S2P_ACT_TANH) stage_out([](float v) { return tanhf(v); });
    else if (a.act == S2P_ACT_SWISH) stage_out([](float v) { return v / (1.f + expf(-v)); });
    else if (a.act == S2P_ACT_NONE) stage_out([](float v) { return v; });
    else {
      const float ns = a.act == S2P_ACT_RELU ? 0.f : a.slope;
      stage_out([ns](float v) { return lrelu_ns(v, ns); });
    }
  };
  if (set == 0) finish(std::integral_constant<int, 0>{}); else finish(std::integral_constant<int, 2>{});
  __syncthreads();
  T* yg = (T*)a.y + (size_t)g * a.y_gstride;
  const T* auxg = a.aux ? (const T*)a.aux + (size_t)g * a.y_gstride : nullptr;
  const T* aux2g = a.aux2 ? (const T*)a.aux2 + (size_t)g * a.y_gstride : nullptr;
  const bool epi_add = a.epi == S2P_EPI_ADD;
  const bool g_tanh = a.gact == S2P_ACT_TANH;
  const float gneg = a.gact == S2P_ACT_RELU ? 0.f : (a.gact == S2P_ACT_LRELU ? a.gslope : 1.f);
  auto out_chunk = [&](int row, int ch, size_t go) {
    Chunk<T> c;
    c.raw = *(const u32x4*)(smem + row * PG_ERS + ch * 16);
    if (a.epi != S2P_EPI_STORE) {
      Chunk<T> x, x2;
      x.raw = *(const u32x4*)(auxg + go);
      x2.raw = (u32x4){0u, 0u, 0u, 0u};
      if (aux2g) x2.raw = *(const u32x4*)(aux2g + go);
      float ov[8];
#pragma unroll
      for (int e = 0; e < 8; ++e) {
        float v = c.get(e), xv = x.get(e);
        const float f = g_tanh ? 1.f - xv * xv : (xv > 0.f ? 1.f : gneg);
        ov[e] = epi_add ? v + xv : (v + x2.get(e)) * f;
      }
      c.pack(ov);
    }
    return c;
  };
  constexpr int MAXR = BPIX / 64;
  if constexpr (MAT == 0) {
    for (int idx = tid; idx < HW * 8; idx += 512) {
      const int row = idx >> 3, ch = idx & 7;
      const size_t go = (pix0 + row) * a.y_pitch + co_base + ch * 8;
      *(u32x4*)(yg + go) = out_chunk(row, ch, go).raw;
    }
  } else if constexpr (MAT == 1) {
    const int ch = tid & 7, r0 = tid >> 3;
    const T* gbb = (GB && a.gb) ? (const T*)a.gb + pix0 * a.gb_pitch + co_base + ch * 8 : nullptr;
    Chunk<T> xv[MAXR], gv[GB ? MAXR : 1], bv[GB ? MAXR : 1];
    if constexpr (GB) {
#pragma unroll
      for (int k = 0; k < MAXR; ++k) {
        const int row = r0 + 64 * k;
        gv[k].raw = (u32x4){0u, 0u, 0u, 0u}; bv[k].raw = gv[k].raw;
        if (gbb && row < HW) {
          gv[k].raw = *(const u32x4*)(gbb + (size_t)row * a.gb_pitch);
          bv[k].raw = *(const u32x4*)(gbb + (size_t)row * a.gb_pitch + a.Cout);
        }
      }
    }
#pragma unroll
    for (int k = 0; k < MAXR; ++k) {
      const int row = r0 + 64 * k;
      xv[k].raw = (u32x4){0u, 0u, 0u, 0u};
      if (row < HW) {
        const size_t go = (pix0 + row) * a.y_pitch + co_base + ch * 8;
        xv[k] = out_chunk(row, ch, go);
        if (a.y) *(u32x4*)(yg + go) = xv[k].raw;
      }
    }
    float xf[MAXR][8];
#pragma unroll
    for (int k = 0; k < MAXR; ++k) xv[k].unpack(xf[k]);
    __syncthreads();
    float* red = (float*)smem;
    float* cst = (float*)smem + 8 * 64;
    auto plane_sum = [&](float (&v)[8], int slot) {
#pragma unroll
      for (int e = 0; e < 8; ++e) {
#pragma unroll
        for (int o = 8; o < 64; o <<= 1) v[e] += __shfl_xor(v[e], o, 64);
      }
      __syncthreads();
      if (lane < 8) {
#pragma unroll
        for (int e = 0; e < 8; ++e) red[wave * 64 + lane * 8 + e] = v[e];
      }
      __syncthreads();
      if (tid < 64) {
        float t = 0.f;
#pragma unroll
        for (int w = 0; w < 8; ++w) t += red[w * 64 + tid];
        cst[slot * 64 + tid] = t;
      }
      __syncthreads();
    };
    const float inv = 1.f / (float)HW;
// ... 119 lines not shown
      const float inv = 1.f / (float)HW;
      cst[4 * 64 + tid] = t0 * inv; cst[5 * 64 + tid] = t1 * inv;
      const int c = co_base + tid;
      if (a.dgbst) {
        a.dgbst[(size_t)img * a.dgbst_pitch + c] = t2;
        a.dgbst[(size_t)img * a.dgbst_pitch + a.Cout + c] = t3;
      }
    }
    __syncthreads();
    T* dxo = (T*)a.y2 + pix0 * a.y2_pitch + lc;
    T* dgo = a.dgb ? (T*)a.dgb + pix0 * a.dgb_pitch + lc : nullptr;
    const T* rsb = a.res ? (const T*)a.res + pix0 * a.res_pitch + lc : nullptr;
    float rr2[8], g12[8], s1v[8], s2v[8];
#pragma unroll
    for (int e = 0; e < 8; ++e) { const int cl = ch * 8 + e; rr2[e] = cst[64 + cl]; g12[e] = cst[128 + cl]; s1v[e] = cst[256 + cl]; s2v[e] = cst[320 + cl]; }
#pragma unroll
    for (int k = 0; k < MAXR; ++k) {
      const int row = r0 + 64 * k;
      if (row >= HW) break;
      Chunk<T> o0, o1, o2;
      float v0[8], v1[8];
#pragma unroll
      for (int e = 0; e < 8; ++e) {
        const float gg = g12[e] + (GB ? gv[k].get(e) : 0.f);
        const float xh = xhf[k][e], dy = dyf[k][e];
        const float dxh = dy * gg;
        v0[e] = rr2[e] * (dxh - s1v[e] - xh * s2v[e]);
        v1[e] = dy * xh;
      }
      o0.pack(v0); o1.pack(v1); o2.pack(dyf[k]);
      if (rsb) {
        Chunk<T> rv; rv.raw = *(const u32x4*)(rsb + (size_t)row * a.res_pitch);
#pragma unroll
        for (int e = 0; e < 8; ++e) v0[e] = o0.get(e) + rv.get(e);
        o0.pack(v0);
      }
      *(u32x4*)(dxo + (size_t)row * a.y2_pitch) = o0.raw;
      if (dgo) {
        *(u32x4*)(dgo + (size_t)row * a.dgb_pitch) = o1.raw;
        *(u32x4*)(dgo + (size_t)row * a.dgb_pitch + a.Cout) = o2.raw;
      }
    }
  }
}

namespace {
struct PgShape { int TY, TX, PB, NPB, S2D; };
const PgShape PG_SHAPES[] = {{4, 4, 1, 128, 0}, {4, 4, 3, 256, 0}, {2, 2, 1, 128, 1}, {2, 2, 3, 256, 1}, {3, 3, 2, 256, 0}, {3, 3, 7, 640, 0},
                             {3, 3, 3, 384, 0}};
constexpr int PG_BAND_SHAPE = 5;
constexpr int PG_BAND_SHAPE_SHORTK = 6;
}

static bool pg_pick_shape(PlaneGArgs& a, int TY, int TX, int s2d, int Cin, int N, bool want_mat) {
  const int HW = a.Ho * a.Wo;
  const int last = (a.Ho - 1 + TY - 1) * a.WP + (a.Wo - 1 + TX - 1);
  a.shape = -1; a.R = a.Ho; a.nbands = 1; a.gimg = 1; a.Hst = 1 << 20;
  if (!s2d && !want_mat && !S2P_DIAG_SWITCH(20)) {
    const int over = TY - 1 - a.PT > a.PT ? TY - 1 - a.PT : a.PT;
    for (int G = 4; G >= 2; G >>= 1) {
      if (N % G || N / G < 16) continue;
      const int Hst = a.Hs + over, lastg = ((G - 1) * Hst + a.Ho - 1 + TY - 1) * a.WP + (a.Wo - 1 + TX - 1);
      for (int i = 0; i < (int)(sizeof(PG_SHAPES) / sizeof(PG_SHAPES[0])); ++i) {
        const PgShape& sh = PG_SHAPES[i];
        if (i == PG_BAND_SHAPE_SHORTK || sh.TY != TY || sh.TX != TX || sh.S2D != s2d) continue;
        if (2 * HW > 4 * sh.PB * 16) break;
        if (G * HW <= 4 * sh.PB * 16 && lastg < sh.NPB) { a.shape = i; a.gimg = G; a.Hst = Hst; return true; }
        break;
      }
    }
  }
  for (int i = 0; i < (int)(sizeof(PG_SHAPES) / sizeof(PG_SHAPES[0])); ++i) {
    const PgShape& s = PG_SHAPES[i];
    if (i != PG_BAND_SHAPE_SHORTK && s.TY == TY && s.TX == TX && s.S2D == s2d && HW <= 4 * s.PB * 16 && last < s.NPB) { a.shape = i; break; }
  }
  if (a.shape >= 0) return 2 * HW > 4 * PG_SHAPES[a.shape].PB * 16;
  if (s2d || S2P_DIAG_SWITCH(4)) return false;
  for (int pass = 0; pass < 2; ++pass) {
    const int bi = pass == 0 ? PG_BAND_SHAPE_SHORTK : PG_BAND_SHAPE;
    if (pass == 0 && (Cin > 64 || S2P_DIAG_SWITCH(8))) continue;
    const PgShape& b = PG_SHAPES[bi];
    if (b.TY != TY || b.TX != TX) continue;
    int R = (b.NPB - TX) / a.WP - (TY - 1);
    if (R * a.Wo > 4 * b.PB * 16) R = (4 * b.PB * 16) / a.Wo;
    if (R < 2 || 4 * R * a.Wo < 3 * 4 * b.PB * 16) continue;
    a.shape = bi; a.R = R; a.nbands = (a.Ho + R - 1) / R;
    return true;
  }
  return false;
}

bool s2p_conv_planeg_setup(const PlaneGProblem& p, PlaneGArgs& a) {
  if (p.Cin % 64 || p.Cout % 64 || p.Cst != p.Cout || p.x_pitch % 8 || p.y_pitch % 8) return false;
  if (p.Ho < 1 || p.Wo < 1) return false;
  if (p.istride == 2) {
    if (p.T != 16) return false;
    for (int t = 0; t < 16; ++t) a.wt[t] = -1;
    for (int t = 0; t < 16; ++t) {
      const int dy = (int)(signed char)(p.tap[t] & 0xff), dx = (int)(signed char)((p.tap[t] >> 8) & 0xff);
      if (dy < -2 || dy > 1 || dx < -2 || dx > 1) return false;
      const int py = dy & 1, px = dx & 1, ra = (dy + 2) >> 1, rb = (dx + 2) >> 1;
      const int k = (py * 2 + px) * 4 + ra * 2 + rb;
      if (a.wt[k] >= 0) return false;
      a.wt[k] = p.tap[t] >> 16;
    }
    a.H = p.Hi; a.W = p.Wi; a.Hs = (p.Hi + 1) / 2; a.Ws = (p.Wi + 1) / 2; a.Ho = p.Ho; a.Wo = p.Wo;
    if (p.Ho != p.Hi / 2 + 1 || p.Wo != p.Wi / 2 + 1) return false;
    a.PT = 1; a.PL = 1;
    const int PR = p.Wo - a.Ws > 0 ? p.Wo - a.Ws : 0;
    a.WP = a.Ws + (PR > 1 ? PR : 1);
    return pg_pick_shape(a, 2, 2, 1, p.Cin, p.N, p.want_mat);
  }
  if (p.istride != 1) return false;
  if (p.T < 1 || p.T > 16) return false;
  int dy0 = 127, dy1 = -127, dx0 = 127, dx1 = -127;
  for (int t = 0; t < p.T; ++t) {
    const int dy = (int)(signed char)(p.tap[t] & 0xff), dx = (int)(signed char)((p.tap[t] >> 8) & 0xff);
    if (dy < dy0) dy0 = dy; if (dy > dy1) dy1 = dy; if (dx < dx0) dx0 = dx; if (dx > dx1) dx1 = dx;
  }
  const int TY = dy1 - dy0 + 1, TX = dx1 - dx0 + 1;
  if (TY * TX != p.T || dy0 > 0 || dx0 > 0) return false;
  for (int t = 0; t < 16; ++t) a.wt[t] = -1;
  for (int t = 0; t < p.T; ++t) {
    const int dy = (int)(signed char)(p.tap[t] & 0xff), dx = (int)(signed char)((p.tap[t] >> 8) & 0xff);
    const int k = (dy - dy0) * TX + (dx - dx0);
    if (a.wt[k] >= 0) return false;
    a.wt[k] = p.tap[t] >> 16;
  }
  a.PT = -dy0; a.PL = -dx0;
  a.H = p.Hi; a.W = p.Wi; a.Hs = p.Hi; a.Ws = p.Wi; a.Ho = p.Ho; a.Wo = p.Wo;
  const int PR = p.Wo - p.Wi + dx1 > 0 ? p.Wo - p.Wi + dx1 : 0;
  a.WP = p.Wi + (a.PL > PR ? a.PL : PR);
  return pg_pick_shape(a, TY, TX, 0, p.Cin, p.N, p.want_mat);
}

template <int TY, int TX, int PB, int NPB, bool S2D>
static void pg_launch_shape(const PlaneGArgs& a, dim3 grid, hipStream_t st) {
  constexpr int RING = (2 * TY * TX) % 8 == 0 ? 8 : 6;
  if (a.y2 && a.xn) hipLaunchKernelGGL((conv_planeg_kernel<TY, TX, PB, NPB, RING, 2, S2D, false>), grid, dim3(512), 0, st, a);
  else if (a.y2) hipLaunchKernelGGL((conv_planeg_kernel<TY, TX, PB, NPB, RING, 1, S2D, false>), grid, dim3(512), 0, st, a);
  else hipLaunchKernelGGL((conv_planeg_kernel<TY, TX, PB, NPB, RING, 0, S2D, false>), grid, dim3(512), 0, st, a);
}

int s2p_conv_planeg_launch(PlaneGArgs& a, int groups, hipStream_t st) {
  a.nco = a.Cout / 64;
  a.img_xcd = (a.N % 8 == 0 && a.nbands > 1 && !S2P_DIAG_SWITCH(15)) ? 1 : 0;
  if (a.gb) S2P_FAIL(-1, "conv_planeg: gamma / beta maps are not instantiated for this kernel family");
  if (a.nbands > 1 && a.y2) S2P_FAIL(-1, "conv_planeg: the fused norm needs the whole plane in one workgroup");
  if (a.gimg > 1 && (a.y2 || a.nbands > 1 || a.N % a.gimg)) S2P_FAIL(-1, "conv_planeg: several images per plane exclude the fused norm and row bands");
  dim3 grid((a.N / a.gimg) * a.nbands * a.nco, groups);
  if (a.shape == 0) pg_launch_shape<4, 4, 1, 128, false>(a, grid, st);
  else if (a.shape == 1) pg_launch_shape<4, 4, 3, 256, false>(a, grid, st);
  else if (a.shape == 2) pg_launch_shape<2, 2, 1, 128, true>(a, grid, st);
  else if (a.shape == 3) pg_launch_shape<2, 2, 3, 256, true>(a, grid, st);
  else if (a.shape == 4) pg_launch_shape<3, 3, 2, 256, false>(a, grid, st);
  else if (a.shape == 5) pg_launch_shape<3, 3, 7, 640, false>(a, grid, st);
  else if (a.shape == 6) pg_launch_shape<3, 3, 3, 384, false>(a, grid, st);
  else S2P_FAIL(-1, "conv_planeg: no kernel instantiated for this shape (s2p_conv_planeg_setup decides)");
  S2P_CHECK_LAUNCH("conv_planeg_kernel");
  return 0;
}
```

### s2p_amd/csrc/misc.hip

```cpp
#include "s2p_common.h"
#include <string.h>

static thread_local char g_err[512] = "";
void s2p_set_error(const char* fmt, ...) {
  va_list ap; va_start(ap, fmt); vsnprintf(g_err, sizeof(g_err), fmt, ap); va_end(ap);
}
extern "C" const char* s2p_last_error(void) { return g_err; }
extern "C" int s2p_version(void) { return S2P_VERSION; }

static inline int grid_for(long long total, int cap = 4096) {
  long long b = (total + 255) / 256; if (b > cap) b = cap; if (b < 1) b = 1; return (int)b;
}
#define GRID_STRIDE(idx, total) \
  for (long long idx = (long long)blockIdx.x * 256 + threadIdx.x; idx < (total); idx += (long long)gridDim.x * 256)

#define S2P_REQUIRE(cond, ...) do { if (!(cond)) S2P_FAIL(-1, __VA_ARGS__); } while (0)
static inline bool is_dtype(int dtype) { return dtype == S2P_F32 || dtype == S2P_BF16; }
static inline bool host_al16(const void* a, const void* b = nullptr, const void* c = nullptr, const void* d = nullptr) {
  return (((uintptr_t)a | (uintptr_t)b | (uintptr_t)c | (uintptr_t)d) & 15) == 0;
}

__global__ void posenc_kernel(const float* s, int N, int S, int L, float* out, int pitch) {
  long long total = (long long)N * pitch;
  GRID_STRIDE(idx, total) {
// ... 162 lines not shown
  long long total = (long long)N * H * W * cpr;
  const bool fast = total < (1ll << 31);
  const IdxDiv dC(cpr, fast), dW(W, fast), dH(H, fast);
  GRID_STRIDE(idx, total) {
    int ch, ix, iy;
    long long p = dC.split(idx, ch);
    p = dW.split(p, ix); int n = (int)dH.split(p, iy);
    int oy = iy >> 1, ox = ix >> 1;
    Chunk<T> o; o.raw = (u32x4){0u, 0u, 0u, 0u};
    if (oy < Ho && ox < Wo) {
      const T* b = x + (((size_t)n * H + oy * 2) * W + ox * 2) * C + ch * CE;
      Chunk<T> v[4], d;
      v[0].raw = *(const u32x4*)b; v[1].raw = *(const u32x4*)(b + C);
      v[2].raw = *(const u32x4*)(b + (size_t)W * C); v[3].raw = *(const u32x4*)(b + (size_t)W * C + C);
      d.raw = *(const u32x4*)(dy + ((((size_t)n * Ho + oy) * Wo + ox) * C + ch * CE));
      const int me = (iy & 1) * 2 + (ix & 1);
      if constexpr (sizeof(T) == 2) {
        typedef __attribute__((ext_vector_type(2))) unsigned short u16x2;
        typedef __attribute__((ext_vector_type(2))) short s16x2;
        const u16x2 one = {1, 1}, zero = {0, 0}, ones = {0xffff, 0xffff};
        const s16x2 szero = {0, 0};
        const bool b0 = me > 0, b1 = me > 1, b2 = me > 2;
#pragma unroll
        for (int j = 0; j < 4; ++j) {
          u16x2 a[4];
#pragma unroll
          for (int k = 0; k < 4; ++k) {
            const unsigned w = v[k].raw[j];
            a[k] = __builtin_bit_cast(u16x2, __builtin_elementwise_max(__builtin_bit_cast(s16x2, w), szero));
          }
          const u16x2 m = __builtin_elementwise_max(__builtin_elementwise_max(a[0], a[1]), __builtin_elementwise_max(a[2], a[3]));
          const u16x2 mine = me == 0 ? a[0] : (me == 1 ? a[1] : (me == 2 ? a[2] : a[3]));
          const u16x2 eq = __builtin_elementwise_min(m - mine, one) - one;
          const u16x2 d0 = b0 ? m - a[0] : ones, d1 = b1 ? m - a[1] : ones, d2 = b2 ? m - a[2] : ones;
          const u16x2 first = zero - __builtin_elementwise_min(__builtin_elementwise_min(__builtin_elementwise_min(d0, d1), d2), one);
          const u16x2 pos = zero - __builtin_elementwise_min(m, one);
          const unsigned dw = d.raw[j];
          o.raw[j] = dw & __builtin_bit_cast(unsigned, eq) & __builtin_bit_cast(unsigned, first) & __builtin_bit_cast(unsigned, pos);
        }
      } else {
        float ov[CE];
#pragma unroll
        for (int e = 0; e < CE; ++e) {
          float m = v[0].get(e); int am = 0;
#pragma unroll
          for (int k = 1; k < 4; ++k) { float t = v[k].get(e); if (t > m) { m = t; am = k; } }
          ov[e] = (am == me && m > 0.f) ? d.get(e) : 0.f;
        }
        o.pack(ov);
      }
    }
    *(u32x4*)(dx + (size_t)idx * CE) = o.raw;
  }
}
extern "C" int s2p_maxpool2x2_fwd(int dtype, const void* x, int N, int H, int W, int C, void* y, void* stream) {
  S2P_REQUIRE(is_dtype(dtype), "s2p_maxpool2x2_fwd: bad dtype");
  S2P_REQUIRE(N >= 0 && H >= 0 && W >= 0 && C >= 0, "s2p_maxpool2x2_fwd: negative size");
  int Ho = H / 2, Wo = W / 2, ce = dtype == S2P_F32 ? 4 : 8;
  if (C % ce) S2P_FAIL(-1, "s2p_maxpool2x2_fwd: C must be a multiple of %d", ce);
  long long total = (long long)N * Ho * Wo * (C / ce);
  if (total == 0) return 0;
  S2P_REQUIRE(x && y, "s2p_maxpool2x2_fwd: null pointer");
  S2P_REQUIRE(host_al16(x, y), "s2p_maxpool2x2_fwd: x and y must be 16-byte aligned");
  if (dtype == S2P_F32) hipLaunchKernelGGL(maxpool_fwd_kernel<float>, dim3(grid_for(total)), dim3(256), 0, (hipStream_t)stream, (const float*)x, N, H, W, C, (float*)y, Ho, Wo);
  else if (dtype == S2P_BF16) hipLaunchKernelGGL(maxpool_fwd_kernel<__bf16>, dim3(grid_for(total)), dim3(256), 0, (hipStream_t)stream, (const __bf16*)x, N, H, W, C, (__bf16*)y, Ho, Wo);
  else S2P_FAIL(-1, "s2p_maxpool2x2_fwd: bad dtype");
  S2P_CHECK_LAUNCH("maxpool_fwd_kernel");
  return 0;
}
extern "C" int s2p_maxpool2x2_bwd(int dtype, const void* dy, const void* x, int N, int H, int W, int C, void* dx, void* stream) {
  S2P_REQUIRE(is_dtype(dtype), "s2p_maxpool2x2_bwd: bad dtype");
  S2P_REQUIRE(N >= 0 && H >= 0 && W >= 0 && C >= 0, "s2p_maxpool2x2_bwd: negative size");
  int Ho = H / 2, Wo = W / 2, ce = dtype == S2P_F32 ? 4 : 8;
  if (C % ce) S2P_FAIL(-1, "s2p_maxpool2x2_bwd: C must be a multiple of %d", ce);
  long long total = (long long)N * H * W * (C / ce);
  if (total == 0) return 0;
  S2P_REQUIRE(x && dx && (dy || (long long)Ho * Wo == 0), "s2p_maxpool2x2_bwd: null pointer");
  S2P_REQUIRE(host_al16(dy, x, dx), "s2p_maxpool2x2_bwd: dy, x and dx must be 16-byte aligned");
  if (dtype == S2P_F32) hipLaunchKernelGGL(maxpool_bwd_kernel<float>, dim3(grid_for(total)), dim3(256), 0, (hipStream_t)stream, (const float*)dy, (const float*)x, N, H, W, C, (float*)dx, Ho, Wo);
  else if (dtype == S2P_BF16) hipLaunchKernelGGL(maxpool_bwd_kernel<__bf16>, dim3(grid_for(total)), dim3(256), 0, (hipStream_t)stream, (const __bf16*)dy, (const __bf16*)x, N, H, W, C, (__bf16*)dx, Ho, Wo);
  else S2P_FAIL(-1, "s2p_maxpool2x2_bwd: bad dtype");
  S2P_CHECK_LAUNCH("maxpool_bwd_kernel");
  return 0;
}

template <typename T>
__global__ void resize_kernel(const T* x, int N, int H, int W, int C, T* y, int Ho, int Wo) {
  long long total = (long long)N * Ho * Wo * C;
  float sy = (float)H / (float)Ho, sx = (float)W / (float)Wo;
  GRID_STRIDE(idx, total) {
    int c = (int)(idx % C); long long p = idx / C;
    int ox = (int)(p % Wo); p /= Wo; int oy = (int)(p % Ho); int n = (int)(p / Ho);
    int iy = (int)floorf(oy * sy), ix = (int)floorf(ox * sx);
    if (iy > H - 1) iy = H - 1; if (ix > W - 1) ix = W - 1;
    y[idx] = x[(((size_t)n * H + iy) * W + ix) * C + c];
  }
}
extern "C" int s2p_resize_nearest(int dtype, const void* x, int N, int H, int W, int C, void* y, int Ho, int Wo, void* stream) {
  S2P_REQUIRE(is_dtype(dtype), "s2p_resize_nearest: bad dtype");
  S2P_REQUIRE(N >= 0 && H >= 0 && W >= 0 && C >= 0 && Ho >= 0 && Wo >= 0, "s2p_resize_nearest: negative size");
  long long total = (long long)N * Ho * Wo * C;
  if (total == 0) return 0;
  S2P_REQUIRE(H > 0 && W > 0, "s2p_resize_nearest: empty input plane");
  S2P_REQUIRE(x && y, "s2p_resize_nearest: null pointer");
  if (dtype == S2P_F32) hipLaunchKernelGGL(resize_kernel<float>, dim3(grid_for(total)), dim3(256), 0, (hipStream_t)stream, (const float*)x, N, H, W, C, (float*)y, Ho, Wo);
  else if (dtype == S2P_BF16) hipLaunchKernelGGL(resize_kernel<__bf16>, dim3(grid_for(total)), dim3(256), 0, (hipStream_t)stream, (const __bf16*)x, N, H, W, C, (__bf16*)y, Ho, Wo);
// ... 774 lines not shown
```

### s2p_amd/csrc/s2p_common.h

```cpp
#pragma once
#include <hip/hip_runtime.h>
#include <stdint.h>
#include <stdio.h>
#include <stdarg.h>
#include <type_traits>
#include "../../include/s2p_hip.h"

typedef __attribute__((ext_vector_type(8))) __bf16 bf16x8;
typedef __attribute__((ext_vector_type(4))) __bf16 bf16x4;
typedef __attribute__((ext_vector_type(16))) float f32x16;
typedef __attribute__((ext_vector_type(4))) float f32x4;
typedef __attribute__((ext_vector_type(4))) short s16x4;
typedef __attribute__((ext_vector_type(4))) unsigned int u32x4;
typedef __attribute__((ext_vector_type(2))) unsigned int u32x2;

#define S2P_WAVE 64

#ifdef S2P_DIAG_BUILD
#include <stdlib.h>
#define S2P_DIAGV(a) ((a).diag)
extern int s2p_diag_switch[32];
#define S2P_DIAG_SWITCH(k) (s2p_diag_switch[k])
static inline int s2p_env_int(const char* name, int dflt) { const char* v = getenv(name); return v ? atoi(v) : dflt; }
static inline int s2p_env_set(const char* name) { return getenv(name) ? 1 : 0; }
// ... 8 lines not shown
#define S2P_FAIL(code, ...) do { s2p_set_error(__VA_ARGS__); return (code); } while (0)
#define S2P_CHECK_SLOPE(who, act, slope) do { if ((act) == S2P_ACT_LRELU && !((slope) <= 1.f)) \
    S2P_FAIL(-1, "%s: leaky-relu slope %g > 1 is not supported", who, (double)(slope)); } while (0)
#define S2P_CHECK_ACT_FROM_OUT(who, act) do { if ((act) != S2P_ACT_NONE && (act) != S2P_ACT_RELU && (act) != S2P_ACT_LRELU && \
    (act) != S2P_ACT_TANH) S2P_FAIL(-1, "%s: no derivative from the output for activation %d (none / relu / lrelu / tanh only)", who, (int)(act)); } while (0)
#define S2P_CHECK_LAUNCH(name) do { hipError_t e_ = hipGetLastError(); \
    if (e_ != hipSuccess) { s2p_set_error("%s: launch failed: %s", name, hipGetErrorString(e_)); \
      return -(int)e_ - 1000; } } while (0)

template <typename T> struct DT;
template <> struct DT<float> { static constexpr int CE = 4; static constexpr int id = S2P_F32; };
template <> struct DT<__bf16> { static constexpr int CE = 8; static constexpr int id = S2P_BF16; };

__device__ __forceinline__ float to_f32(float v) { return v; }
__device__ __forceinline__ float to_f32(__bf16 v) { return (float)v; }
template <typename T> __device__ __forceinline__ T from_f32(float v);
template <> __device__ __forceinline__ float from_f32<float>(float v) { return v; }
template <> __device__ __forceinline__ __bf16 from_f32<__bf16>(float v) { return (__bf16)v; }

template <typename T> struct Chunk;
template <> struct Chunk<float> {
  u32x4 raw;
  __device__ __forceinline__ float get(int i) const { unsigned u = raw[i]; return __uint_as_float(u); }
  __device__ __forceinline__ void set(int i, float v) { unsigned u = __float_as_uint(v); raw[i] = u; }
  __device__ __forceinline__ void unpack(float (&v)[4]) const { for (int e = 0; e < 4; ++e) v[e] = get(e); }
  __device__ __forceinline__ void pack(const float (&v)[4]) { for (int e = 0; e < 4; ++e) set(e, v[e]); }
};
template <> struct Chunk<__bf16> {
  u32x4 raw;
  __device__ __forceinline__ float get(int i) const {
    unsigned w = raw[i >> 1];
    unsigned b = (i & 1) ? (w & 0xffff0000u) : (w << 16);
    return __builtin_bit_cast(float, b);
  }
  __device__ __forceinline__ void set(int i, float v) {
    __bf16 h = (__bf16)v;
    unsigned short u = __builtin_bit_cast(unsigned short, h);
    unsigned w = raw[i >> 1];
    raw[i >> 1] = (i & 1) ? ((w & 0x0000ffffu) | ((unsigned)u << 16)) : ((w & 0xffff0000u) | u);
  }
  __device__ __forceinline__ void unpack(float (&v)[8]) const {
#pragma unroll
    for (int e = 0; e < 8; ++e) v[e] = get(e);
  }
  __device__ __forceinline__ void pack(const float (&v)[8]) {
    typedef __attribute__((ext_vector_type(2))) __bf16 bf16x2_t;
#pragma unroll
    for (int e = 0; e < 4; ++e) {
      const bf16x2_t h = {(__bf16)v[2 * e], (__bf16)v[2 * e + 1]};
      raw[e] = __builtin_bit_cast(unsigned, h);
    }
  }
};

__device__ __forceinline__ double s2p_rcp_f64(int d) {
  const double x = (double)d;
  double r = __builtin_amdgcn_rcp(x);
  r = __builtin_fma(__builtin_fma(-x, r, 1.0), r, r);
  r = __builtin_fma(__builtin_fma(-x, r, 1.0), r, r);
  return r;
}
__device__ __forceinline__ int divmod_rcp(int m, int d, double rcp, int& rem) {
  int q = (int)((double)m * rcp);
  int r = m - q * d;
  const int lo = r < 0 ? 1 : 0;
  q -= lo; r += lo ? d : 0;
  const int hi = r >= d ? 1 : 0;
  q += hi; r -= hi ? d : 0;
  rem = r;
  return q;
}
struct IdxDiv {
  int d; double r; bool fast;
  __device__ __forceinline__ IdxDiv(int d_, bool fast_) : d(d_), r(fast_ ? s2p_rcp_f64(d_) : 0.0), fast(fast_) {}
  __device__ __forceinline__ long long split(long long idx, int& rem) const {
    if (fast) return divmod_rcp((int)idx, d, r, rem);
    const long long q = idx / d; rem = (int)(idx - q * d); return q;
  }
};

__device__ __forceinline__ float lrelu_ns(float v, float ns) {
  const float m = v * ns;
  float r;
  asm("v_max_f32 %0, %1, %2" : "=v"(r) : "v"(v), "v"(m));
  return r;
}

__device__ __forceinline__ float act_fwd(float v, int act, float slope) {
  switch (act) {
    case S2P_ACT_RELU: return v > 0.f ? v : 0.f;
    case S2P_ACT_LRELU: return v > 0.f ? v : v * slope;
    case S2P_ACT_TANH: return tanhf(v);
    case S2P_ACT_SWISH: return v / (1.f + expf(-v));
    default: return v;
  }
}
__device__ __forceinline__ float act_grad_from_out(float y, int act, float slope) {
  switch (act) {
    case S2P_ACT_RELU: return y > 0.f ? 1.f : 0.f;
    case S2P_ACT_LRELU: return y > 0.f ? 1.f : slope;
    case S2P_ACT_TANH: return 1.f - y * y;
    default: return 1.f;
  }
}

__device__ __forceinline__ float lds_ld(const float* p) {
// ... 106 lines not shown
```

### s2p_amd/models/autograd_nodes.py

```python
import torch

from .. import ops, stepgraph
from .._lib import chunk_elems


DBWD_LANE = 0
OVERLAP_VGG = True


def _vgg_stream(model):
    s = getattr(model, "_vgg_side", None)
    if s is None:
        s = model._vgg_side = torch.cuda.Stream()
    return s


def _anchor(net):
    a = getattr(net, "_anchor", None)
    if a is None or a.device != net.store.master.device:
        a = torch.zeros(1, device=net.store.master.device, requires_grad=True)
        net._anchor = a
    return a


# ... 12 lines not shown
            raise RuntimeError("generator forward was run without saving activations")
        ctx.net.bwd_nhwc(ctx.c, d_out.contiguous())
        ctx.c = None
        return None, None, None, None, None


def generator_apply(net, prev_image, state):
    save = torch.is_grad_enabled()
    return _GeneratorNode.apply(_anchor(net) if save else _anchor(net).detach(), prev_image, state, net, save)


class _NhwcToNchw(torch.autograd.Function):
    @staticmethod
    def forward(ctx, x, C):
        ctx.dt, ctx.pitch = x.dtype, x.shape[3]
        return ops.nhwc_to_nchw(x, C)

    @staticmethod
    def backward(ctx, g):
        return ops.nchw_to_nhwc(g.contiguous().float(), ctx.dt, ctx.pitch), None


def nhwc_to_nchw_apply(x, C):
    return _NhwcToNchw.apply(x, C)


def _build_d_half(model, prev_image, image_nchw=None, image_nhwc=None):
    dt = model.netD.compute_dtype
    N, _, H, W = prev_image.shape
    x = torch.empty((N, H, W, 8), dtype=dt, device=prev_image.device)
    ops.nchw_to_nhwc(prev_image, dt, 8, out=x, c_off=0, zero_pad=True)
    if image_nhwc is not None:
        ops.copy_channels(image_nhwc, 0, x, 3, 3, src_rows=N)
    else:
        ops.nchw_to_nhwc(image_nchw, dt, 8, out=x, c_off=3, zero_pad=False)
    return x


def _side(model, name):
    s = getattr(model, name, None)
    if s is None:
        s = torch.cuda.Stream()
        setattr(model, name, s)
    return s


def vgg_real_prefetch(model, real_image, dt, ce):
    main = torch.cuda.current_stream()
    vs = _vgg_stream(model)
    stepgraph.fork(vs, main)
    real_image.record_stream(vs)
    with torch.cuda.stream(vs):
        real_nhwc = ops.nchw_to_nhwc(real_image, dt, ce)
        taps, acts = model.vgg.fwd_nhwc(real_nhwc)
    return dict(real_nhwc=real_nhwc, taps=taps, acts=acts, stream=vs)


OVERLAP_DREAL = True
DREAL_EARLY_BWD = True
DREAL_REUSE = True


def _dreal_key(model, prev_image, real_image):
    return (id(prev_image), prev_image._version, prev_image.data_ptr(), id(real_image), real_image._version,
            real_image.data_ptr(), getattr(model.netD.store, "version", 0))


def _record_ctx(dctx, stream):
    for x, saved in dctx:
        x.record_stream(stream)
        for tup in saved:
            for t in tup:
                if t is not None:
                    t.record_stream(stream)


def dreal_pass(model, prev_image, real_image, on_side):
    main = torch.cuda.current_stream()
    side = _side(model, "_dreal_side") if on_side else main
    if on_side:
        stepgraph.fork(side, main)
        prev_image.record_stream(side); real_image.record_stream(side)
    with torch.cuda.stream(side):
        xr = _build_d_half(model, prev_image, image_nchw=real_image)
        res, dctx = model.netD.fwd_nhwc(xr, lane=None if on_side else 0)
    if on_side:
        _record_ctx(dctx, main)
    return dict(res=res, dctx=dctx, stream=side if on_side else None, key=_dreal_key(model, prev_image, real_image))


def _hinge_seed(logits, mode, N, num_D, loss_slot):
    B, h, w, ce = logits.shape
    return ops.hinge_loss_nhwc(logits, mode, 1.0 / (N * h * w * num_D), loss_slot)


class _GLossNode(torch.autograd.Function):

    @staticmethod
    def forward(ctx, fake, model, prev_image, real_image, pre, pre_d):
        opt = model.opt
        N, H, W, ce = fake.shape
        dt = fake.dtype
        main = torch.cuda.current_stream()
        if pre is not None:
            main.wait_stream(pre["stream"])
        if pre_d is not None and pre_d["stream"] is not None:
            main.wait_stream(pre_d["stream"])
        if model.before_netD is not None:
            model.before_netD()
        losses = torch.zeros(4, dtype=torch.float32, device=fake.device)
        real_nhwc = pre["real_nhwc"] if pre is not None else ops.nchw_to_nhwc(real_image, dt, ce)
        d_fake = torch.zeros_like(fake)
        if opt.lambda_l1 > 0:
            ops.l1_loss(fake, real_nhwc, opt.lambda_l1 / (N * 3 * H * W), losses[3:4], d_fake)
        vgg_on_side = (not opt.no_vgg_loss) and OVERLAP_VGG and not ops.SERIALIZE
        vs = _vgg_stream(model) if vgg_on_side else main
        vctx, tap_grads, vctx_real = None, None, None
        if not opt.no_vgg_loss:
            from .networks.loss import VGG_WEIGHTS
            if vgg_on_side:
                stepgraph.fork(vs, main)
                fake.record_stream(vs); losses.record_stream(vs); real_nhwc.record_stream(vs)
            with torch.cuda.stream(vs):
                if pre is not None:
                    taps_r, vctx_real = pre["taps"], pre["acts"]
                else:
                    taps_r, vctx_real = model.vgg.fwd_nhwc(real_nhwc)
                taps, vctx = model.vgg.fwd_nhwc(fake)
                tap_grads = [torch.empty_like(t) for t in taps]
                ops.l1_loss_multi([(t, tr, opt.lambda_vgg * wk / t.numel(), losses[2:3], tg)
                                   for wk, t, tr, tg in zip(VGG_WEIGHTS, taps, taps_r, tap_grads)])
        dreal = pre_d
        if dreal is None:
            model.netD.sn_forward()
            dreal = dreal_pass(model, prev_image, real_image, OVERLAP_DREAL and not ops.SERIALIZE)
        xf = _build_d_half(model, prev_image, image_nhwc=fake)
        res, dctx = model.netD.fwd_nhwc(xf)
        if pre_d is None and dreal["stream"] is not None:
            main.wait_stream(dreal["stream"])
        res_r = dreal["res"]
        model._dreal_cache = dreal
        num_D = len(res)
        grads, fm_jobs = [], []
        for feats, feats_r in zip(res, res_r):
            g = [None] * len(feats)
            g[-1] = _hinge_seed(feats[-1], 2, N, num_D, losses[0:1])
            if not opt.no_ganFeat_loss:
                for j in range(len(feats) - 1):
                    f = feats[j]
                    gf = torch.empty_like(f)
                    fm_jobs.append((f, feats_r[j], opt.lambda_feat / num_D / f.numel(), losses[1:2], gf))
                    g[j] = gf
            grads.append(g)
        if fm_jobs:
            ops.l1_loss_multi(fm_jobs)
        if vgg_on_side:
            main.wait_stream(vs)
        ctx.vgg_on_side = vgg_on_side
        ctx.model, ctx.dctx, ctx.grads, ctx.vctx, ctx.tap_grads, ctx.d_fake, ctx.N = \
            model, dctx, grads, vctx, tap_grads, d_fake, N
        ctx.dctx_r = dreal["dctx"]
        ctx.vctx_real, ctx.real_nhwc, ctx.fake = vctx_real, real_nhwc, fake
        return tuple(losses.unbind(0))

    @staticmethod
    def backward(ctx, *gs_in):
        model, N = ctx.model, ctx.N
        if not model.assume_unit_loss_grad:
            g = torch.stack([gi.float() if gi is not None else torch.zeros((), device=ctx.d_fake.device) for gi in gs_in])
            for gs in ctx.grads:
                ops.scale_(gs[-1], g[0:1])
                for t in gs[:-1]:
                    if t is not None:
                        ops.scale_(t, g[1:2])
            if ctx.tap_grads is not None:
                for t in ctx.tap_grads:
                    ops.scale_(t, g[2:3])
            ops.scale_(ctx.d_fake, g[3:4])
        d_fake = ctx.d_fake
        main = torch.cuda.current_stream()
# ... 106 lines not shown
```

### s2p_amd/models/networks/layers.py

```python
import torch
import torch.nn as nn

from ... import ops
from ..._lib import ACT_LRELU, ACT_NONE, ACT_RELU, ACT_TANH, EPI_ADD, EPI_MUL_ACTGRAD, EPI_STORE, chunk_elems
from ...ops import ConvGeom, pad_to


class ConvLayer:

    def __init__(self, packed, geom, cin_real=None, cout_real=None):
        self.pk, self.geom = packed, geom
        self.cin_real = cin_real if cin_real is not None else geom.cin
        self.cout_real = cout_real if cout_real is not None else geom.cout

    def cin_pad(self, dtype):
        return pad_to(self.geom.cin, chunk_elems(dtype))

    def fwd(self, x, act=ACT_NONE, slope=0.2, aux=None, epi=EPI_STORE, y_pitch=None):
        return ops.conv_fwd(self.geom, x, self.pk.w_fwd, self.pk.bias, self.cin_pad(x.dtype), y_pitch=y_pitch,
                            act=act, slope=slope, aux=aux, epi=epi)

    def _group_major(self, t5):
        g = self.geom
        assert t5.dim() == 5 and t5.shape[0] == g.groups and t5.is_contiguous()
        key = t5.stride(0)
        gm = self.__dict__.setdefault("_gm", {})
        if key not in gm:
            gm[key] = ConvGeom(g.cin, g.cout, g.k, g.stride, g.pad, g.transposed, g.reflect, g.groups, g.output_padding,
                               x_gstride=g.x_gstride, y_gstride=key, net=g.net)
        return gm[key]

    def fwd_group_major(self, x, out5):
        gm = self._group_major(out5)
        ops.conv_fwd(gm, x, self.pk.w_fwd, self.pk.bias, self.cin_pad(x.dtype), y_pitch=out5.shape[4], out=out5[0])
        return out5

    def fwd_mat(self, x, gb, gb_off, gb_st, st_off, act, slope, aux=None, epi=EPI_STORE, want_y=True):
        return ops.conv_fwd_mat(self.geom, x, self.pk.w_fwd, self.pk.bias, self.cin_pad(x.dtype), gb, gb_off, gb_st, st_off,
                                act=act, slope=slope, aux=aux, epi=epi, want_y=want_y)

    def dgrad(self, dy, x_shape, aux=None, epi=EPI_STORE, aux_act=ACT_NONE, slope=0.2, aux2=None):
        if dy.dim() == 5:
            return ops.conv_dgrad(self._group_major(dy), dy[0], self.pk.w_bwd, tuple(x_shape), self.cin_pad(dy.dtype), aux=aux,
                                  epi=epi, aux_act=aux_act, slope=slope, aux2=aux2)
        return ops.conv_dgrad(self.geom, dy, self.pk.w_bwd, tuple(x_shape), self.cin_pad(dy.dtype), aux=aux, epi=epi,
                              aux_act=aux_act, slope=slope, aux2=aux2)

    def dgrad_mat(self, dy, xn, stats, gb, gb_off, gb_st, st_off, act, slope, dgb, dgb_off, dgb_st, dst_off, res=None, aux=None):
        return ops.conv_dgrad_mat(self.geom, dy, self.pk.w_bwd, xn, self.cin_pad(dy.dtype), stats, gb, gb_off, gb_st, st_off,
                                  act, slope, dgb, dgb_off, dgb_st, dst_off, res=res, aux=aux)

    def wgrad(self, x, dy, groups=None):
        g = self.geom
        if g.groups > 1 and x.dtype == torch.bfloat16 and g.k == 3 and g.stride == 1 and g.pad == 1 and not g.transposed \
                and g.groups <= 16 and g.cin % 64 == 0 and g.cout % 64 == 0:
            one = ConvGeom(g.cin, g.cout, 3, 1, 1, net=g.net)
            gw = self.pk.gw.view(g.groups, -1)
            gb = self.pk.gb.view(g.groups, -1) if self.pk.gb is not None else None
            sel = range(g.groups) if groups is None else range(groups[0], groups[1])
            if dy.dim() == 5:
                jobs = [(x, i * g.x_gstride, dy[i], 0, gw[i], gb[i] if gb is not None else None) for i in sel]
            else:
                jobs = [(x, i * g.x_gstride, dy, i * g.y_gstride, gw[i], gb[i] if gb is not None else None) for i in sel]
            ops.conv_wgrad_batched(one, jobs, g.cin, self.cin_real, self.cout_real)
            return
        if groups is not None:
            raise RuntimeError("a group range is only wired for the batched slab weight-gradient path")
        if dy.dim() == 5:
            raise RuntimeError("group-major dY is only wired for the batched slab weight-gradient path (bf16, 3x3, 64-channel multiples)")
        if g.groups == 1 and g.cout == 1 and x.dtype == torch.bfloat16 and g.stride == 1 and not g.transposed and not g.reflect:
            ops.conv_wgrad_batched(g, [(x, 0, dy, 0, self.pk.gw, self.pk.gb)], self.cin_pad(x.dtype), self.cin_real,
                                   self.cout_real)
            return
# ... 22 lines not shown
```

### s2p_amd/models/networks/loss.py

```python
import torch
import torch.nn as nn

from ... import ops
from ..._lib import ACT_RELU, EPI_MUL_ACTGRAD, chunk_elems
from ...ops import ConvGeom
from .base_network import BaseNetwork
from .generator import _Conv
from .layers import ConvLayer

VGG_CFG = [("conv1_1", 3, 64), ("conv1_2", 64, 64), "P",
           ("conv2_1", 64, 128), ("conv2_2", 128, 128), "P",
           ("conv3_1", 128, 256), ("conv3_2", 256, 256), ("conv3_3", 256, 256), ("conv3_4", 256, 256), "P",
           ("conv4_1", 256, 512), ("conv4_2", 512, 512), ("conv4_3", 512, 512), ("conv4_4", 512, 512), "P",
           ("conv5_1", 512, 512)]
VGG_TAPS = ("conv1_1", "conv2_1", "conv3_1", "conv4_1", "conv5_1")
VGG_WEIGHTS = (1.0 / 32, 1.0 / 16, 1.0 / 8, 1.0 / 4, 1.0)
TORCHVISION_IDX = dict(conv1_1=0, conv1_2=2, conv2_1=5, conv2_2=7, conv3_1=10, conv3_2=12, conv3_3=14, conv3_4=16,
                       conv4_1=19, conv4_2=21, conv4_3=23, conv4_4=25, conv5_1=28)


class VGG19(BaseNetwork):
    def __init__(self, opt=None):
        super().__init__()
        for item in VGG_CFG:
            if item != "P":
                name, cin, cout = item
                setattr(self, name, _Conv(cin, cout, 3, bias=True))
        for p in self.parameters():
            p.requires_grad_(False)

    def init_standin(self, seed=1234):
        g = torch.Generator().manual_seed(seed)
        with torch.no_grad():
            for name, p in self.named_parameters():
                if name.endswith(".bias"):
                    p.zero_()
                else:
                    fan_in = p.shape[1] * p.shape[2] * p.shape[3]
                    p.copy_(torch.randn(p.shape, generator=g) * (2.0 / fan_in) ** 0.5)
        if self.finalized:
            self.store.repack()

    def load_torchvision(self, path):
        sd = torch.load(path, map_location="cpu")
        mine = {}
        for name, idx in TORCHVISION_IDX.items():
            for suffix in ("weight", "bias"):
                for key in (f"features.{idx}.{suffix}", f"{idx}.{suffix}", f"{name}.{suffix}"):
                    if key in sd:
                        mine[f"{name}.{suffix}"] = sd[key]
                        break
        self.load_state_dict(mine, strict=True)

    def _declare_packs(self, dt):
        self.lay = {}
        for item in VGG_CFG:
            if item == "P":
                continue
            name, cin, cout = item
            m = getattr(self, name)
            self.store.add(m.weight, "conv"); self.store.add(m.bias, "bias")
            pk = self.store.pack(name, [m.weight], [m.bias], dtype=dt)
            self.lay[name] = ConvLayer(pk, ConvGeom(cin, cout, 3, 1, 1, net="VGG"))

    def fwd_nhwc(self, x):
        self._require_ready()
        acts = []
        h = x
        taps = []
        for item in VGG_CFG:
            if item == "P":
                o = ops.maxpool_fwd(h)
                acts.append(("P", None, h, o))
            else:
                name = item[0]
                o = self.lay[name].fwd(h, act=ACT_RELU)
                acts.append(("C", name, h, o))
                if name in VGG_TAPS:
                    taps.append(o)
            h = o
        return taps, acts

    def bwd_nhwc(self, acts, tap_grads, n_fake):
        tapg = dict(zip(VGG_TAPS, tap_grads))
        d = None
        for kind, name, xin, out in reversed(acts):
            xin_f, out_f = xin[:n_fake], out[:n_fake]
            if kind == "P":
                d = ops.maxpool_bwd(d, xin_f)
                continue
            if d is None:
                d = ops.act_bwd(tapg[name], out_f, ACT_RELU)
            lay = self.lay[name]
            if name == "conv1_1":
                return lay.dgrad(d, xin_f.shape)
            prev_is_pool = self._prev_kind(acts, name) == "P"
            if prev_is_pool:
                d = lay.dgrad(d, xin_f.shape)
            else:
                prev_name = self._prev_name(acts, name)
                d = lay.dgrad(d, xin_f.shape, aux=xin_f, epi=EPI_MUL_ACTGRAD, aux_act=ACT_RELU,
                              aux2=tapg.get(prev_name))
        raise RuntimeError("unreachable")

    @staticmethod
    def _prev_kind(acts, name):
        for i, (kind, n, _, _) in enumerate(acts):
            if n == name:
                return acts[i - 1][0] if i > 0 else None
        return None

    @staticmethod
    def _prev_name(acts, name):
        for i, (kind, n, _, _) in enumerate(acts):
            if n == name:
                return acts[i - 1][1] if i > 0 else None
        return None
```

### s2p_amd/ops.py

```python
import ctypes

import torch

from . import _lib
from ._lib import (ACT_LRELU, ACT_NONE, ACT_RELU, ACT_TANH, EPI_ADD, EPI_MUL_ACTGRAD, EPI_STORE, ConvDesc,
                   check, chunk_elems, dtype_id, lib, ptr, stream)

IN_EPS = 1e-5

SERIALIZE = False


PROFILE = None


class _Prof:
    def __init__(self, kind, geom, N, H, W, dtype):
        self.on = PROFILE is not None
        if self.on:
            Ho, Wo = geom.out_hw(H, W)
            pix = N * H * W if geom.transposed else N * Ho * Wo
            self.rec = dict(kind=kind, flops=2.0 * pix * geom.cin * geom.cout * geom.k * geom.k * geom.groups,
                            shape=(N, H, W, geom.cin, geom.cout, geom.k, geom.stride, geom.groups, int(geom.transposed)),
                            dtype=str(dtype), net=getattr(geom, "net", ""))
# ... 24 lines not shown
            self.e1.record()
            self.rec["events"] = (self.e0, self.e1)
            PROFILE.append(self.rec)


def pad_to(c, ce):
    return (c + ce - 1) // ce * ce


_MAT_FUSED = {}
SKIP_UNUSED_Y = True


class ConvGeom:

    def __init__(self, cin, cout, k, stride=1, pad=0, transposed=False, reflect=False, groups=1,
                 output_padding=0, x_gstride=0, y_gstride=0, net=""):
        self.net = net
        self.cin, self.cout, self.k = cin, cout, k
        self.stride, self.pad = stride, pad
        self.transposed, self.reflect, self.groups = transposed, reflect, groups
        self.output_padding = output_padding
        self.x_gstride, self.y_gstride = x_gstride, y_gstride

    def out_hw(self, H, W):
        k, s, p = self.k, self.stride, self.pad
        if self.transposed:
            return ((H - 1) * s - 2 * p + k + self.output_padding, (W - 1) * s - 2 * p + k + self.output_padding)
        return ((H + 2 * p - k) // s + 1, (W + 2 * p - k) // s + 1)

    def desc(self, dtype, N, H, W, cin_pad, x_pitch, y_pitch):
        Ho, Wo = self.out_hw(H, W)
        return ConvDesc(dtype_id(dtype), N, H, W, cin_pad, x_pitch, Ho, Wo, self.cout, y_pitch,
                        self.k, self.k, self.stride, self.pad, int(self.transposed), int(self.reflect),
                        self.groups, self.x_gstride, self.y_gstride, self.cin if self.groups == 1 else 0)


def conv_fwd(geom, x, w_fwd, bias, cin_pad, y_pitch=None, act=ACT_NONE, slope=0.2, aux=None, epi=EPI_STORE,
             out=None):
    N, H, W, xp = x.shape
    ce = chunk_elems(x.dtype)
    Ho, Wo = geom.out_hw(H, W)
    if y_pitch is None:
        y_pitch = pad_to(geom.cout * geom.groups if geom.groups > 1 else geom.cout, ce)
    y = out if out is not None else torch.empty((N, Ho, Wo, y_pitch), dtype=x.dtype, device=x.device)
    d = geom.desc(x.dtype, N, H, W, cin_pad, xp, y_pitch)
    need = lib().s2p_conv2d_fwd_workspace(ctypes.byref(d), epi)
    ws = torch.empty(need, dtype=torch.uint8, device=x.device) if need else None
    pr = _Prof("fwd", geom, N, H, W, x.dtype)
    check(lib().s2p_conv2d_fwd_ws(ctypes.byref(d), ptr(x), ptr(w_fwd), ptr(bias), ptr(aux), ptr(y), act, slope, epi,
                                  ptr(ws), need, stream()), "s2p_conv2d_fwd")
    pr.done()
    return y


def conv_fwd_mat(geom, x, w_fwd, bias, cin_pad, gb, gb_off, gb_st, st_off, act=ACT_LRELU, slope=0.2, aux=None, epi=EPI_STORE,
                 want_y=True):
    N, H, W, xp = x.shape
    Ho, Wo = geom.out_hw(H, W)
    C = geom.cout
    y_pitch = pad_to(C, chunk_elems(x.dtype))
    y_mat = torch.empty((N, Ho, Wo, C), dtype=x.dtype, device=x.device)
    stats = torch.empty(lib().s2p_in_stats_floats(N, Ho * Wo, C), dtype=torch.float32, device=x.device)
    d = geom.desc(x.dtype, N, H, W, cin_pad, xp, y_pitch)
    y = None
    if not SKIP_UNUSED_Y:
        want_y = True
    if not want_y:
        key = (geom.cin, geom.cout, geom.k, geom.stride, geom.pad, geom.transposed, geom.reflect, geom.groups, geom.output_padding,
               x.dtype, N, H, W, cin_pad, xp, gb is not None)
        if key not in _MAT_FUSED:
            _MAT_FUSED[key] = bool(lib().s2p_conv2d_mat_is_fused(ctypes.byref(d), 0, 1 if gb is not None else 0))
        want_y = not _MAT_FUSED[key]
    if want_y:
        y = torch.empty((N, Ho, Wo, y_pitch), dtype=x.dtype, device=x.device)
    need = lib().s2p_conv2d_fwd_workspace(ctypes.byref(d), epi)
    ws = torch.empty(need, dtype=torch.uint8, device=x.device) if need else None
    gbp, gb_pitch, stp, st_pitch = _gb_args(gb, gb_off, gb_st, st_off)
    pr = _Prof("fwd", geom, N, H, W, x.dtype)
    if pr.on:
        pr.rec["norm_bytes"] = float(N * Ho * Wo * C * x.element_size() * 3)
        pr.rec["variant"] = "mat_fwd"
    check(lib().s2p_conv2d_fwd_mat(ctypes.byref(d), ptr(x), ptr(w_fwd), ptr(bias), ptr(aux), ptr(y), epi, gbp, gb_pitch, stp,
                                   st_pitch, act, slope, IN_EPS, ptr(y_mat), C, ptr(stats), ptr(ws), need, stream()),
          "s2p_conv2d_fwd_mat")
    pr.done()
    return y, y_mat, stats


def conv_dgrad(geom, dy, w_bwd, x_shape, cin_pad, aux=None, epi=EPI_STORE, aux_act=ACT_NONE, slope=0.2, aux2=None):
    N, H, W, xp = x_shape
    d = geom.desc(dy.dtype, N, H, W, cin_pad, xp, dy.shape[3])
    if geom.reflect:
        p = geom.pad
        dxp = torch.empty((N, H + 2 * p, W + 2 * p, xp), dtype=dy.dtype, device=dy.device)
        need = lib().s2p_conv2d_dgrad_workspace(ctypes.byref(d))
        ws = torch.empty(need, dtype=torch.uint8, device=dy.device) if need else None
        pr = _Prof("dgrad", geom, N, H, W, dy.dtype)
        check(lib().s2p_conv2d_dgrad_ws(ctypes.byref(d), ptr(dy), ptr(w_bwd), None, None, ptr(dxp), EPI_STORE, ACT_NONE, 0.0,
                                        ptr(ws), need, stream()), "s2p_conv2d_dgrad")
        pr.done()
        dx = torch.empty((N, H, W, xp), dtype=dy.dtype, device=dy.device)
        check(lib().s2p_reflect_pad_bwd(dtype_id(dy.dtype), ptr(dxp), N, H, W, xp, p, ptr(dx), stream()),
              "s2p_reflect_pad_bwd")
        if aux2 is not None:
            dx = add(dx, aux2, out=dx)
# ... 167 lines not shown
                               n_store, stream()), "s2p_linear_fwd")
    return y


def linear_bwd(x, dy, y, w_bwd, K, k_real, N, act, slope, dw, db, need_dx=True):
    M, xp = x.shape
    dx = torch.empty((M, xp), dtype=torch.float32, device=x.device) if need_dx else None
    need = lib().s2p_linear_bwd_workspace(M, K, N) if need_dx else 0
    ws = torch.empty(max(need, 16), dtype=torch.uint8, device=x.device)
    check(lib().s2p_linear_bwd(ptr(x), xp, ptr(dy), dy.shape[1], ptr(y), y.shape[1] if y is not None else 0, M, K, k_real, N,
                               ptr(w_bwd), w_bwd.shape[-1] if w_bwd is not None else 0, act, slope, ptr(dw), k_real, ptr(db),
                               ptr(dx), xp, ptr(ws), need, stream()), "s2p_linear_bwd")
    return dx


def posenc(state, L, pitch):
    N, S = state.shape
    out = torch.empty((N, pitch), dtype=torch.float32, device=state.device)
    check(lib().s2p_posenc_fwd(ptr(state), N, S, L, ptr(out), pitch, stream()), "s2p_posenc_fwd")
    return out


def avgpool_fwd(x):
    N, H, W, C = x.shape
    y = torch.empty((N, (H - 1) // 2 + 1, (W - 1) // 2 + 1, C), dtype=x.dtype, device=x.device)
    check(lib().s2p_avgpool3x3s2_fwd(dtype_id(x.dtype), ptr(x), N, H, W, C, ptr(y), stream()), "s2p_avgpool3x3s2_fwd")
    return y


def avgpool_bwd(dy, x_shape, dx=None, accumulate=False):
    N, H, W, C = x_shape
    if dx is None:
        dx = torch.empty(x_shape, dtype=dy.dtype, device=dy.device)
    check(lib().s2p_avgpool3x3s2_bwd(dtype_id(dy.dtype), ptr(dy), N, H, W, C, ptr(dx), int(accumulate), stream()),
          "s2p_avgpool3x3s2_bwd")
    return dx


def maxpool_fwd(x):
    N, H, W, C = x.shape
    y = torch.empty((N, H // 2, W // 2, C), dtype=x.dtype, device=x.device)
    check(lib().s2p_maxpool2x2_fwd(dtype_id(x.dtype), ptr(x), N, H, W, C, ptr(y), stream()), "s2p_maxpool2x2_fwd")
    return y


def maxpool_bwd(dy, x):
    N, H, W, C = x.shape
    dx = torch.empty_like(x)
    check(lib().s2p_maxpool2x2_bwd(dtype_id(x.dtype), ptr(dy), ptr(x), N, H, W, C, ptr(dx), stream()),
          "s2p_maxpool2x2_bwd")
    return dx


def resize_nearest(x, Ho, Wo):
    N, H, W, C = x.shape
    y = torch.empty((N, Ho, Wo, C), dtype=x.dtype, device=x.device)
    check(lib().s2p_resize_nearest(dtype_id(x.dtype), ptr(x), N, H, W, C, ptr(y), Ho, Wo, stream()), "s2p_resize_nearest")
    return y


def nchw_to_nhwc(x, dtype, pitch, out=None, c_off=0, zero_pad=True):
    N, C, H, W = x.shape
    x = x.contiguous()
    y = out if out is not None else torch.empty((N, H, W, pitch), dtype=dtype, device=x.device)
    check(lib().s2p_nchw_to_nhwc(dtype_id(dtype), ptr(x), N, C, H, W, ptr(y), pitch, c_off, int(zero_pad), stream()),
          "s2p_nchw_to_nhwc")
    return y


def nhwc_to_nchw(x, C, c_off=0, out=None, accumulate=False):
    N, H, W, xp = x.shape
    y = out if out is not None else torch.empty((N, C, H, W), dtype=torch.float32, device=x.device)
    if not y.is_contiguous() or tuple(y.shape) != (N, C, H, W) or y.dtype != torch.float32:
        raise ValueError("nhwc_to_nchw: `out` must be a contiguous fp32 [N,C,H,W] tensor, got shape %s strides %s %s" % (
            tuple(y.shape), y.stride(), y.dtype))
    check(lib().s2p_nhwc_to_nchw(dtype_id(x.dtype), ptr(x), xp, c_off, N, C, H, W, ptr(y), int(accumulate), stream()),
          "s2p_nhwc_to_nchw")
    return y


def cast(x, dtype):
    y = torch.empty(x.shape, dtype=dtype, device=x.device)
    check(lib().s2p_cast(dtype_id(x.dtype), ptr(x), dtype_id(dtype), ptr(y), x.numel(), stream()), "s2p_cast")
    return y


def act_bwd(dy, y, act, slope=0.2):
    dx = torch.empty_like(dy)
    check(lib().s2p_act_bwd(dtype_id(dy.dtype), ptr(dy), ptr(y), dy.numel(), act, slope, ptr(dx), stream()), "s2p_act_bwd")
    return dx


def scale_(x, scale_dev):
    check(lib().s2p_scale(dtype_id(x.dtype), ptr(x), x.numel(), ptr(scale_dev), stream()), "s2p_scale")
    return x


def l1_loss(a, b, scale, loss_out, grad_a=None, accumulate=False):
    check(lib().s2p_l1_loss(dtype_id(a.dtype), ptr(a), ptr(b), a.numel(), scale, ptr(loss_out), ptr(grad_a),
                            int(accumulate), stream()), "s2p_l1_loss")


def l1_loss_multi(jobs):
    cap = 16
    for i0 in range(0, len(jobs), cap):
        part = jobs[i0:i0 + cap]
# ... 144 lines not shown
```

Baseline: 8083 images/sec.

## Fuse 2x2 maxpool into VGG conv epilogue with argmax index for backward

Adds a pooled epilogue to the plane and plane-pair conv kernels, so VGG convs that feed a maxpool write the pooled output and a per-element argmax code straight from shared memory. When the full-resolution activation is not needed, it is never written. The VGG forward uses this for non-tap convs before pools, and the backward uses a new index-based maxpool backward. The real-image VGG pass skips storing indices. This removes a full-resolution activation write and read plus a separate pool kernel, at the cost of extra kernel template variants and an index buffer.

```diff
diff --git a/include/s2p_hip.h b/include/s2p_hip.h
--- a/include/s2p_hip.h
+++ b/include/s2p_hip.h
@@ -54,6 +54,9 @@
                          void* dgb_img, int dgb_pitch, float* dgb_st, int dgb_st_pitch, const void* res, int res_pitch,
                          void* workspace, size_t workspace_bytes, void* stream);
 int s2p_conv2d_mat_is_fused(const s2p_conv_desc* d, int dgrad, int has_gb);
+int s2p_conv2d_fwd_can_pool(const s2p_conv_desc* d, int act);
+int s2p_conv2d_fwd_pool(const s2p_conv_desc* d, const void* x, const void* w_fwd, const float* bias, void* y, void* pool_y,
+                        void* pool_idx, int act, void* stream);
 int s2p_conv2d_wgrad(const s2p_conv_desc* d, const void* x, const void* dy, float* dw, float* db,
                      int cin_real, int cout_real, int64_t dw_gstride, int splitk, void* stream);
 size_t s2p_conv2d_wgrad_workspace(const s2p_conv_desc* d, int cin_real, int cout_real);
@@ -140,6 +143,8 @@
 int s2p_maxpool2x2_fwd(int dtype, const void* x, int N, int H, int W, int C, void* y, void* stream);
 int s2p_maxpool2x2_bwd(int dtype, const void* dy, const void* x, int N, int H, int W, int C,
                        void* dx, void* stream);
+int s2p_maxpool2x2_bwd_idx(int dtype, const void* dy, const void* pool_y, const void* pool_idx, int N, int H, int W, int C,
+                           void* dx, void* stream);
 int s2p_resize_nearest(int dtype, const void* x, int N, int H, int W, int C, void* y, int Ho, int Wo,
                        void* stream);
 int s2p_nchw_to_nhwc(int dtype, const float* x, int N, int C, int H, int W, void* y, int y_pitch,
diff --git a/s2p_amd/_lib.py b/s2p_amd/_lib.py
--- a/s2p_amd/_lib.py
+++ b/s2p_amd/_lib.py
@@ -55,6 +55,8 @@
     "s2p_conv2d_dgrad_mat": [_DESC, _P, _P, _P, _P, _P, c_int, _P, _P, c_int, _P, c_int, c_int, c_float, c_float, _P, _P, c_int, _P, c_int,
                              _P, c_int, _P, c_int, _P, ctypes.c_size_t, _P],
     "s2p_conv2d_mat_is_fused": [_DESC, c_int, c_int],
+    "s2p_conv2d_fwd_can_pool": [_DESC, c_int],
+    "s2p_conv2d_fwd_pool": [_DESC, _P, _P, _P, _P, _P, _P, c_int, _P],
     "s2p_conv2d_dgrad_workspace": [_DESC],
     "s2p_conv2d_dgrad_ws": [_DESC, _P, _P, _P, _P, _P, c_int, c_int, c_float, _P, ctypes.c_size_t, _P],
     "s2p_conv2d_wgrad": [_DESC, _P, _P, _P, _P, c_int, c_int, c_int64, c_int, _P],
@@ -99,6 +101,7 @@
     "s2p_avgpool3x3s2_bwd": [c_int, _P, c_int, c_int, c_int, c_int, _P, c_int, _P],
     "s2p_maxpool2x2_fwd": [c_int, _P, c_int, c_int, c_int, c_int, _P, _P],
     "s2p_maxpool2x2_bwd": [c_int, _P, _P, c_int, c_int, c_int, c_int, _P, _P],
+    "s2p_maxpool2x2_bwd_idx": [c_int, _P, _P, _P, c_int, c_int, c_int, c_int, _P, _P],
     "s2p_resize_nearest": [c_int, _P, c_int, c_int, c_int, c_int, _P, c_int, c_int, _P],
     "s2p_nchw_to_nhwc": [c_int, _P, c_int, c_int, c_int, c_int, _P, c_int, c_int, c_int, _P],
     "s2p_nhwc_to_nchw": [c_int, _P, c_int, c_int, c_int, c_int, c_int, c_int, _P, c_int, _P],
diff --git a/s2p_amd/csrc/conv_igemm.hip b/s2p_amd/csrc/conv_igemm.hip
--- a/s2p_amd/csrc/conv_igemm.hip
+++ b/s2p_amd/csrc/conv_igemm.hip
@@ -1189,7 +1189,8 @@
   const void* x; const void* w; const float* bias; const void* aux; const void* aux2; void* y;
   int act; float slope; int epi, gact; float gslope;
 };
-struct NormWant { bool any, gb, bwd; };
+struct NormWant { bool any, gb, bwd; bool pool = false; };
+struct PoolOut { void* y; void* idx; };
 struct ScratchAvail { bool any; size_t bytes; };
 static const ScratchAvail SCRATCH_UNLIMITED{true, ~(size_t)0};
 struct Scratch { void* ws; size_t bytes; };
@@ -1197,6 +1198,7 @@
 struct GatherChoice {
   ConvPath path = ConvPath::Generic;
   bool fused = false;
+  bool pooled = false;
   size_t ws_bytes = 0;
   int bco = 128;
   HaloKind halo = HaloKind::R_320;
@@ -1206,7 +1208,7 @@
 struct GatherItem { GatherArgs a; GatherChoice c; };
 struct ConvPlan {
   ConvPath path = ConvPath::Generic;
-  bool fused = false;
+  bool fused = false, pooled = false;
   size_t ws_bytes = 0;
   int cout_pad = 0;
   std::vector<GatherItem> items;
@@ -1215,6 +1217,7 @@
     if (it.c.ws_bytes > ws_bytes) ws_bytes = it.c.ws_bytes;
     items.push_back(it);
     fused = items.size() == 1 && it.c.fused;
+    pooled = items.size() == 1 && it.c.pooled;
   }
 };
 
@@ -1244,6 +1247,7 @@
   const int nwg = a.npix_tiles * a.nco_tiles;
   const bool whole = a.ostride == 1 && a.oy0 == 0 && a.ox0 == 0 && a.Qh == a.Ho && a.Qw == a.Wo;
   const bool planes = whole && a.M % (a.Qh * a.Qw) == 0;
+  const bool pool_ok = want.pool && !want.any && groups == 1 && a.act == S2P_ACT_RELU && a.epi == S2P_EPI_STORE && a.T == 9 && a.istride == 1;
   int S = 1;
   if (!sw.no_dma && !sw.no_split && groups == 1 && whole && sc.any) S = conv_split_plan(nwg, a.Ktot / 64);
   if (!sw.no_plane && !sw.no_dma && a.T == 9 && a.istride == 1 && planes && a.Qh == a.Hi && a.Qw == a.Wi) {
@@ -1260,17 +1264,19 @@
     if (ok && s2p_conv_plane_applicable(p)) {
       c.path = ConvPath::Plane;
       c.fused = want.any && groups == 1 && a.act == S2P_ACT_NONE && a.epi != S2P_EPI_MUL_ACTGRAD && (!want.bwd || a.epi == S2P_EPI_STORE);
+      c.pooled = pool_ok;
       return;
     }
   }
   if (!sw.no_plane && !sw.no_planeg() && !(a.T == 9 && sw.no_planeg_3x3()) && !sw.no_dma && groups == 1 && planes && !a.reflect) {
-    PlaneGProblem pr{a.M / (a.Qh * a.Qw), a.Hi, a.Wi, a.Ho, a.Wo, a.Cin, a.Cout, a.Cst, a.x_pitch, a.y_pitch, a.istride, a.T, a.tap, want.any};
+    PlaneGProblem pr{a.M / (a.Qh * a.Qw), a.Hi, a.Wi, a.Ho, a.Wo, a.Cin, a.Cout, a.Cst, a.x_pitch, a.y_pitch, a.istride, a.T, a.tap, want.any, pool_ok};
     PlaneGArgs& p = c.planeg;
     if (s2p_conv_planeg_setup(pr, p)) {
       copy_conv_fields(p, a);
       p.N = pr.N;
       c.path = ConvPath::PlaneG;
       c.fused = want.any && p.nbands == 1 && p.gimg == 1 && !want.gb && a.act == S2P_ACT_NONE && a.epi != S2P_EPI_MUL_ACTGRAD;
+      c.pooled = pool_ok && p.gimg == 1 && (p.nbands == 1 || (p.R & 1) == 0);
       return;
     }
   }
@@ -1515,14 +1521,16 @@
   return launch_cfg<T, 32, 256, 1, 4>(a, groups, st);
 }
 
-static int launch_item(GatherItem& it, bool bf16, int groups, const PlaneMat* mat, void* ws, hipStream_t st) {
+static int launch_item(GatherItem& it, bool bf16, int groups, const PlaneMat* mat, const PoolOut* pool, void* ws, hipStream_t st) {
   if (!bf16) return launch_generic<float>(it.a, groups, st);
   switch (it.c.path) {
     case ConvPath::Plane:
       if (it.c.fused) copy_norm(it.c.plane, *mat);
+      if (it.c.pooled) { it.c.plane.pool_y = pool->y; it.c.plane.pool_idx = pool->idx; }
       return s2p_conv_plane_launch(it.c.plane, groups, st);
     case ConvPath::PlaneG:
       if (it.c.fused) copy_norm(it.c.planeg, *mat);
+      if (it.c.pooled) { it.c.planeg.pool_y = pool->y; it.c.planeg.pool_idx = pool->idx; }
       return s2p_conv_planeg_launch(it.c.planeg, groups, st);
     case ConvPath::Phases: {
       GatherArgs& a = it.a;
@@ -1539,30 +1547,32 @@
   }
   return launch_generic<__bf16>(it.a, groups, st);
 }
-static int launch_items(ConvPlan& P, bool bf16, int groups, const PlaneMat* mat, const Scratch& sc, hipStream_t st) {
+static int launch_items(ConvPlan& P, bool bf16, int groups, const PlaneMat* mat, const PoolOut* pool, const Scratch& sc, hipStream_t st) {
   for (GatherItem& it : P.items) {
-    const int rc = launch_item(it, bf16, groups, mat, sc.ws, st);
+    const int rc = launch_item(it, bf16, groups, mat, pool, sc.ws, st);
     if (rc) return rc;
   }
   return 0;
 }
 
-static int conv_fwd_impl(const s2p_conv_desc* d, const ConvOperands& op, const PlaneMat* mat, bool* fused, const Scratch& sc, void* stream) {
+static int conv_fwd_impl(const s2p_conv_desc* d, const ConvOperands& op, const PlaneMat* mat, bool* fused, const Scratch& sc, void* stream,
+                         const PoolOut* pool = nullptr) {
   S2P_CHECK_SLOPE("s2p_conv2d_fwd", op.act, op.slope);
   if (mat) S2P_CHECK_SLOPE("s2p_conv2d_fwd_mat", mat->act, mat->slope);
   ConvPlan P;
-  int rc = conv_plan_fwd(d, op, NormWant{mat != nullptr, mat && mat->gb, false}, ScratchAvail{sc.ws != nullptr, sc.bytes}, P);
+  int rc = conv_plan_fwd(d, op, NormWant{mat != nullptr, mat && mat->gb, false, pool != nullptr}, ScratchAvail{sc.ws != nullptr, sc.bytes}, P);
   if (rc) return rc;
-  if (!op.x || !op.w || (!op.y && !mat)) S2P_FAIL(-1, "s2p_conv2d_fwd: null pointer");
+  if (!op.x || !op.w || (!op.y && !mat && !pool)) S2P_FAIL(-1, "s2p_conv2d_fwd: null pointer");
   if (op.epi != S2P_EPI_STORE && !op.aux) S2P_FAIL(-1, "s2p_conv2d_fwd: epi needs aux");
-  if (!op.y && !P.fused) S2P_FAIL(-1, "s2p_conv2d_fwd_mat: y == NULL needs the fused launch (s2p_conv2d_mat_is_fused)");
+  if (pool && !P.pooled) S2P_FAIL(-1, "s2p_conv2d_fwd_pool: no kernel with the pooled epilogue takes this problem (s2p_conv2d_fwd_can_pool)");
+  if (!op.y && !pool && !P.fused) S2P_FAIL(-1, "s2p_conv2d_fwd_mat: y == NULL needs the fused launch (s2p_conv2d_mat_is_fused)");
   if (fused) *fused = P.fused;
   hipStream_t st = (hipStream_t)stream;
   switch (P.path) {
     case ConvPath::Thin: return s2p_thin_fwd(d, op.x, op.w, op.bias, op.y, op.act, op.slope, st);
     case ConvPath::Thin4: return s2p_thin4_fwd(d, op.x, op.w, op.bias, op.y, op.act, op.slope, sc.ws, sc.bytes, st);
     case ConvPath::ThinCin: return s2p_thin_cin_fwd(d, op.x, op.w, op.bias, op.y, op.act, op.slope, st);
-    default: return launch_items(P, d->dtype == S2P_BF16, d->groups, mat, sc, st);
+    default: return launch_items(P, d->dtype == S2P_BF16, d->groups, mat, pool, sc, st);
   }
 }
 
@@ -1590,6 +1600,20 @@
   if (rc || fused) return rc;
   return s2p_in_norm_fwd(d->dtype, y, d->N, d->Ho * d->Wo, d->Cout, d->y_pitch, gb_img, gb_pitch, gb_st, gb_st_pitch, act, slope,
                          eps, y_mat, y_mat_pitch, stats, stream);
+}
+extern "C" int s2p_conv2d_fwd_can_pool(const s2p_conv_desc* d, int act) {
+  if (!d || d->groups != 1 || d->transposed || d->reflect) return 0;
+  const ConvOperands op{nullptr, nullptr, nullptr, nullptr, nullptr, nullptr, act, 0.f, S2P_EPI_STORE, S2P_ACT_NONE, 0.f};
+  ConvPlan P;
+  return conv_plan_fwd(d, op, NormWant{false, false, false, true}, ScratchAvail{false, 0}, P) == 0 && P.pooled ? 1 : 0;
+}
+extern "C" int s2p_conv2d_fwd_pool(const s2p_conv_desc* d, const void* x, const void* w_fwd, const float* bias, void* y, void* pool_y,
+                                   void* pool_idx, int act, void* stream) {
+  if (!d || !pool_y) S2P_FAIL(-1, "s2p_conv2d_fwd_pool: null pointer");
+  if ((((uintptr_t)pool_y | (uintptr_t)pool_idx) & 15) != 0) S2P_FAIL(-1, "s2p_conv2d_fwd_pool: pool_y and pool_idx must be 16-byte aligned");
+  const PoolOut pool{pool_y, pool_idx};
+  return conv_fwd_impl(d, ConvOperands{x, w_fwd, bias, nullptr, nullptr, y, act, 0.f, S2P_EPI_STORE, 0, 0.f}, nullptr, nullptr, Scratch{nullptr, 0},
+                       stream, &pool);
 }
 extern "C" size_t s2p_conv2d_fwd_workspace(const s2p_conv_desc* d, int epi) {
   ConvPlan P;
@@ -1613,7 +1637,7 @@
   switch (P.path) {
     case ConvPath::Thin4: return s2p_thin4_dgrad(d, op.x, op.w, op.y, P.cout_pad, sc.ws, sc.bytes, st);
     case ConvPath::ThinRows: return s2p_thin_rows_dgrad(d, op.x, op.w, op.y, P.cout_pad, st);
-    default: return launch_items(P, d->dtype == S2P_BF16, d->groups, mat, sc, st);
+    default: return launch_items(P, d->dtype == S2P_BF16, d->groups, mat, nullptr, sc, st);
   }
 }
 
diff --git a/s2p_amd/csrc/conv_plane.h b/s2p_amd/csrc/conv_plane.h
--- a/s2p_amd/csrc/conv_plane.h
+++ b/s2p_amd/csrc/conv_plane.h
@@ -24,6 +24,7 @@
   const void* xn; int xn_pitch; void* dgb; int dgb_pitch; float* dgbst; int dgbst_pitch; const void* res; int res_pitch;
   int nco, gxcd;
   int diag;
+  void* pool_y; void* pool_idx;
 };
 
 bool s2p_conv_plane_applicable(const PlaneArgs& a);
diff --git a/s2p_amd/csrc/conv_plane.hip b/s2p_amd/csrc/conv_plane.hip
--- a/s2p_amd/csrc/conv_plane.hip
+++ b/s2p_amd/csrc/conv_plane.hip
@@ -18,9 +18,10 @@
 constexpr int PL_ERS = 144;
 }
 
-template <int PB, int WP, int DIAG, int MAT = 0, int GST = 0>
+template <int PB, int WP, int DIAG, int MAT = 0, int GST = 0, int POOL = 0>
 __global__ __launch_bounds__(512) void conv_plane_kernel(const PlaneArgs a) {
   typedef __bf16 T;
+  static_assert(POOL == 0 || (MAT == 0 && DIAG == 0), "pooled epilogue: plain product kernel only");
   static_assert(GST == 0 || (MAT != 0 && DIAG == 0 && PB == 7), "gamma|beta staging: fused-norm product kernels only");
   constexpr int BPIX = 4 * PB * 16;
   constexpr int NT = 4 * PB;
@@ -401,10 +402,28 @@
     return c;
   };
   if constexpr (MAT == 0) {
-    for (int idx = tid; idx < HW * 8; idx += 512) {
-      const int row = idx >> 3, ch = idx & 7;
-      const size_t go = ((size_t)img * HW + row) * a.y_pitch + co_base + ch * 8;
-      *(u32x4*)(yg + go) = out_chunk(row, ch, go).raw;
+    if (POOL == 0 || a.y) {
+      for (int idx = tid; idx < HW * 8; idx += 512) {
+        const int row = idx >> 3, ch = idx & 7;
+        const size_t go = ((size_t)img * HW + row) * a.y_pitch + co_base + ch * 8;
+        *(u32x4*)(yg + go) = out_chunk(row, ch, go).raw;
+      }
+    }
+    if constexpr (POOL != 0) {
+      const int Hp = a.H >> 1, Wp = a.W >> 1;
+      const float rwp = 1.0f / (float)(Wp > 0 ? Wp : 1);
+      for (int idx = tid; idx < Hp * Wp * 8; idx += 512) {
+        const int pp = idx >> 3, ch = idx & 7;
+        const int oy = (int)(((float)pp + 0.5f) * rwp), ox = pp - oy * Wp;
+        const int r00 = 2 * oy * a.W + 2 * ox;
+        Chunk<T> v[4], o; u32x2 code;
+        v[0].raw = *(const u32x4*)srow(r00, ch); v[1].raw = *(const u32x4*)srow(r00 + 1, ch);
+        v[2].raw = *(const u32x4*)srow(r00 + a.W, ch); v[3].raw = *(const u32x4*)srow(r00 + a.W + 1, ch);
+        pool2x2_chunk(v, o, code);
+        const size_t po = ((size_t)img * Hp * Wp + pp) * a.y_pitch + co_base + ch * 8;
+        *(u32x4*)((T*)a.pool_y + po) = o.raw;
+        if (a.pool_idx) *(u32x2*)((unsigned char*)a.pool_idx + po) = code;
+      }
     }
   } else if constexpr (MAT == 1) {
     constexpr int MAXR = BPIX / 64;
@@ -668,7 +687,7 @@
   }
 }
 
-template <int PB, int WP, int DIAG>
+template <int PB, int WP, int DIAG, int POOL = 0>
 __global__ __launch_bounds__(512) void conv_plane_pair_kernel(const PlaneArgs a) {
   typedef __bf16 T;
   constexpr int BPIX = 4 * PB * 16;
@@ -858,7 +877,8 @@
     const bool epi_add = a.epi == S2P_EPI_ADD;
     const bool g_tanh = a.gact == S2P_ACT_TANH;
     const float gneg = a.gact == S2P_ACT_RELU ? 0.f : (a.gact == S2P_ACT_LRELU ? a.gslope : 1.f);
-    for (int idx = tid; idx < HW * 16; idx += 512) {
+    const int nstore = (POOL == 0 || a.y) ? HW * 16 : 0;
+    for (int idx = tid; idx < nstore; idx += 512) {
       const int row = idx >> 4, ch16 = idx & 15, sl = ch16 >> 3, ch = ch16 & 7;
       Chunk<T> c;
       c.raw = *(const u32x4*)(smem + sl * EPI + row * PL_ERS + ch * 16);
@@ -879,6 +899,22 @@
       }
       *(u32x4*)(yg + go) = c.raw;
     }
+    if constexpr (POOL != 0) {
+      const int Hp = a.H >> 1, Wp = a.W >> 1;
+      const float rwp = 1.0f / (float)(Wp > 0 ? Wp : 1);
+      for (int idx = tid; idx < Hp * Wp * 16; idx += 512) {
+        const int pp = idx >> 4, ch16 = idx & 15, sl = ch16 >> 3, ch = ch16 & 7;
+        const int oy = (int)(((float)pp + 0.5f) * rwp), ox = pp - oy * Wp;
+        const char* b = smem + sl * EPI + (2 * oy * a.W + 2 * ox) * PL_ERS + ch * 16;
+        Chunk<T> v[4], o; u32x2 code;
+        v[0].raw = *(const u32x4*)b; v[1].raw = *(const u32x4*)(b + PL_ERS);
+        v[2].raw = *(const u32x4*)(b + a.W * PL_ERS); v[3].raw = *(const u32x4*)(b + (a.W + 1) * PL_ERS);
+        pool2x2_chunk(v, o, code);
+        const size_t po = ((size_t)img * Hp * Wp + pp) * a.y_pitch + (2 * cpair + sl) * 64 + ch * 8;
+        *(u32x4*)((T*)a.pool_y + po) = o.raw;
+        if (a.pool_idx) *(u32x2*)((unsigned char*)a.pool_idx + po) = code;
+      }
+    }
   }
 }
 
@@ -894,6 +930,7 @@
 int s2p_conv_plane_launch(PlaneArgs& a, int groups, hipStream_t st) {
   a.nco = a.Cout / 64;
   dim3 grid(a.N * a.nco, groups);
+  if (a.pool_y && (a.y2 || groups != 1 || a.epi != S2P_EPI_STORE)) S2P_FAIL(-1, "conv_plane: the pooled epilogue takes a plain conv, groups == 1");
 #ifdef S2P_DIAG_BUILD
   static const int diag = s2p_env_int("S2P_DIAG", 0);
 #define PL_DIAG_CASE(D) if (diag == D) { hipLaunchKernelGGL((conv_plane_kernel<7, 22, D>), grid, dim3(512), 0, st, a); S2P_CHECK_LAUNCH("conv_plane_kernel(diag)"); return 0; }
@@ -903,7 +940,8 @@
   if (!a.y2 && (a.nco & 1) == 0 && (long long)a.N * a.nco * groups > 256 && !s2p_env_set("S2P_NO_PLANE_PAIR")) {
     dim3 gp(a.N * (a.nco / 2), groups);
     a.gxcd = (groups > 1 && (2 * groups) % 8 == 0 && a.N % 2 == 0 && gp.x % 8 == 0 && !S2P_DIAG_SWITCH(17)) ? 1 : 0;
-    hipLaunchKernelGGL((conv_plane_pair_kernel<7, 22, 0>), gp, dim3(512), 0, st, a);
+    if (a.pool_y) hipLaunchKernelGGL((conv_plane_pair_kernel<7, 22, 0, 1>), gp, dim3(512), 0, st, a);
+    else hipLaunchKernelGGL((conv_plane_pair_kernel<7, 22, 0>), gp, dim3(512), 0, st, a);
     S2P_CHECK_LAUNCH("conv_plane_pair_kernel");
     return 0;
   }
@@ -918,7 +956,8 @@
     else hipLaunchKernelGGL((conv_plane_kernel<7, 22, 0, 1>), grid, dim3(512), 0, st, a);
     S2P_CHECK_LAUNCH("conv_plane_kernel(mat)"); return 0;
   }
-  hipLaunchKernelGGL((conv_plane_kernel<7, 22, 0>), grid, dim3(512), 0, st, a);
+  if (a.pool_y) hipLaunchKernelGGL((conv_plane_kernel<7, 22, 0, 0, 0, 1>), grid, dim3(512), 0, st, a);
+  else hipLaunchKernelGGL((conv_plane_kernel<7, 22, 0>), grid, dim3(512), 0, st, a);
   S2P_CHECK_LAUNCH("conv_plane_kernel");
   return 0;
 }
diff --git a/s2p_amd/csrc/conv_planeg.h b/s2p_amd/csrc/conv_planeg.h
--- a/s2p_amd/csrc/conv_planeg.h
+++ b/s2p_amd/csrc/conv_planeg.h
@@ -25,12 +25,14 @@
   int R, nbands;
   int shape;
   int gimg, Hst;
+  void* pool_y; void* pool_idx;
 };
 
 struct PlaneGProblem {
   int N, Hi, Wi, Ho, Wo, Cin, Cout, Cst, x_pitch, y_pitch, istride, T;
   const int* tap;
   bool want_mat;
+  bool want_pool;
 };
 bool s2p_conv_planeg_setup(const PlaneGProblem& p, PlaneGArgs& a);
 int s2p_conv_planeg_launch(PlaneGArgs& a, int groups, hipStream_t st);
diff --git a/s2p_amd/csrc/conv_planeg.hip b/s2p_amd/csrc/conv_planeg.hip
--- a/s2p_amd/csrc/conv_planeg.hip
+++ b/s2p_amd/csrc/conv_planeg.hip
@@ -313,11 +313,30 @@
     return c;
   };
   constexpr int MAXR = BPIX / 64;
-  if constexpr (MAT == 0) {
-    for (int idx = tid; idx < HW * 8; idx += 512) {
-      const int row = idx >> 3, ch = idx & 7;
-      const size_t go = (pix0 + row) * a.y_pitch + co_base + ch * 8;
-      *(u32x4*)(yg + go) = out_chunk(row, ch, go).raw;
+  if constexpr (MAT == 0 || MAT == 3) {
+    if (MAT == 0 || a.y) {
+      for (int idx = tid; idx < HW * 8; idx += 512) {
+        const int row = idx >> 3, ch = idx & 7;
+        const size_t go = (pix0 + row) * a.y_pitch + co_base + ch * 8;
+        *(u32x4*)(yg + go) = out_chunk(row, ch, go).raw;
+      }
+    }
+    if constexpr (MAT == 3) {
+      const int Wp = a.Wo >> 1, nr = rows_here >> 1;
+      const float rwp = 1.0f / (float)(Wp > 0 ? Wp : 1);
+      const size_t pp0 = ((size_t)img * (a.Ho >> 1) + (r0 >> 1)) * Wp;
+      for (int idx = tid; idx < nr * Wp * 8; idx += 512) {
+        const int pp = idx >> 3, ch = idx & 7;
+        const int oy = (int)(((float)pp + 0.5f) * rwp), ox = pp - oy * Wp;
+        const char* b = smem + (2 * oy * a.Wo + 2 * ox) * PG_ERS + ch * 16;
+        Chunk<T> v[4], o; u32x2 code;
+        v[0].raw = *(const u32x4*)b; v[1].raw = *(const u32x4*)(b + PG_ERS);
+        v[2].raw = *(const u32x4*)(b + a.Wo * PG_ERS); v[3].raw = *(const u32x4*)(b + (a.Wo + 1) * PG_ERS);
+        pool2x2_chunk(v, o, code);
+        const size_t po = (pp0 + pp) * a.y_pitch + co_base + ch * 8;
+        *(u32x4*)((T*)a.pool_y + po) = o.raw;
+        if (a.pool_idx) *(u32x2*)((unsigned char*)a.pool_idx + po) = code;
+      }
     }
   } else if constexpr (MAT == 1) {
     const int ch = tid & 7, r0 = tid >> 3;
@@ -543,11 +562,11 @@
 constexpr int PG_BAND_SHAPE_SHORTK = 6;
 }
 
-static bool pg_pick_shape(PlaneGArgs& a, int TY, int TX, int s2d, int Cin, int N, bool want_mat) {
+static bool pg_pick_shape(PlaneGArgs& a, int TY, int TX, int s2d, int Cin, int N, bool want_mat, bool want_pool) {
   const int HW = a.Ho * a.Wo;
   const int last = (a.Ho - 1 + TY - 1) * a.WP + (a.Wo - 1 + TX - 1);
   a.shape = -1; a.R = a.Ho; a.nbands = 1; a.gimg = 1; a.Hst = 1 << 20;
-  if (!s2d && !want_mat && !S2P_DIAG_SWITCH(20)) {
+  if (!s2d && !want_mat && !want_pool && !S2P_DIAG_SWITCH(20)) {
     const int over = TY - 1 - a.PT > a.PT ? TY - 1 - a.PT : a.PT;
     for (int G = 4; G >= 2; G >>= 1) {
       if (N % G || N / G < 16) continue;
@@ -574,6 +593,7 @@
     if (b.TY != TY || b.TX != TX) continue;
     int R = (b.NPB - TX) / a.WP - (TY - 1);
     if (R * a.Wo > 4 * b.PB * 16) R = (4 * b.PB * 16) / a.Wo;
+    if (want_pool) R &= ~1;
     if (R < 2 || 4 * R * a.Wo < 3 * 4 * b.PB * 16) continue;
     a.shape = bi; a.R = R; a.nbands = (a.Ho + R - 1) / R;
     return true;
@@ -600,7 +620,7 @@
     a.PT = 1; a.PL = 1;
     const int PR = p.Wo - a.Ws > 0 ? p.Wo - a.Ws : 0;
     a.WP = a.Ws + (PR > 1 ? PR : 1);
-    return pg_pick_shape(a, 2, 2, 1, p.Cin, p.N, p.want_mat);
+    return pg_pick_shape(a, 2, 2, 1, p.Cin, p.N, p.want_mat, false);
   }
   if (p.istride != 1) return false;
   if (p.T < 1 || p.T > 16) return false;
@@ -622,12 +642,15 @@
   a.H = p.Hi; a.W = p.Wi; a.Hs = p.Hi; a.Ws = p.Wi; a.Ho = p.Ho; a.Wo = p.Wo;
   const int PR = p.Wo - p.Wi + dx1 > 0 ? p.Wo - p.Wi + dx1 : 0;
   a.WP = p.Wi + (a.PL > PR ? a.PL : PR);
-  return pg_pick_shape(a, TY, TX, 0, p.Cin, p.N, p.want_mat);
+  return pg_pick_shape(a, TY, TX, 0, p.Cin, p.N, p.want_mat, p.want_pool);
 }
 
 template <int TY, int TX, int PB, int NPB, bool S2D>
 static void pg_launch_shape(const PlaneGArgs& a, dim3 grid, hipStream_t st) {
   constexpr int RING = (2 * TY * TX) % 8 == 0 ? 8 : 6;
+  if constexpr (TY == 3 && TX == 3 && !S2D) {
+    if (a.pool_y) { hipLaunchKernelGGL((conv_planeg_kernel<TY, TX, PB, NPB, RING, 3, S2D, false>), grid, dim3(512), 0, st, a); return; }
+  }
   if (a.y2 && a.xn) hipLaunchKernelGGL((conv_planeg_kernel<TY, TX, PB, NPB, RING, 2, S2D, false>), grid, dim3(512), 0, st, a);
   else if (a.y2) hipLaunchKernelGGL((conv_planeg_kernel<TY, TX, PB, NPB, RING, 1, S2D, false>), grid, dim3(512), 0, st, a);
   else hipLaunchKernelGGL((conv_planeg_kernel<TY, TX, PB, NPB, RING, 0, S2D, false>), grid, dim3(512), 0, st, a);
@@ -639,6 +662,8 @@
   if (a.gb) S2P_FAIL(-1, "conv_planeg: gamma / beta maps are not instantiated for this kernel family");
   if (a.nbands > 1 && a.y2) S2P_FAIL(-1, "conv_planeg: the fused norm needs the whole plane in one workgroup");
   if (a.gimg > 1 && (a.y2 || a.nbands > 1 || a.N % a.gimg)) S2P_FAIL(-1, "conv_planeg: several images per plane exclude the fused norm and row bands");
+  if (a.pool_y && (a.shape < 4 || a.y2 || a.gimg > 1 || groups != 1 || a.epi != S2P_EPI_STORE || (a.nbands > 1 && (a.R & 1))))
+    S2P_FAIL(-1, "conv_planeg: the pooled epilogue takes a plain 3x3 conv, groups == 1, one image per plane, bands of an even row count");
   dim3 grid((a.N / a.gimg) * a.nbands * a.nco, groups);
   if (a.shape == 0) pg_launch_shape<4, 4, 1, 128, false>(a, grid, st);
   else if (a.shape == 1) pg_launch_shape<4, 4, 3, 256, false>(a, grid, st);
diff --git a/s2p_amd/csrc/misc.hip b/s2p_amd/csrc/misc.hip
--- a/s2p_amd/csrc/misc.hip
+++ b/s2p_amd/csrc/misc.hip
@@ -238,6 +238,53 @@
     }
     *(u32x4*)(dx + (size_t)idx * CE) = o.raw;
   }
+}
+template <typename T>
+__global__ void maxpool_bwd_idx_kernel(const T* dy, const T* py, const unsigned char* code, int N, int H, int W, int C, T* dx, int Ho, int Wo) {
+  constexpr int CE = DT<T>::CE;
+  int cpr = C / CE;
+  long long total = (long long)N * H * W * cpr;
+  const bool fast = total < (1ll << 31);
+  const IdxDiv dC(cpr, fast), dW(W, fast), dH(H, fast);
+  GRID_STRIDE(idx, total) {
+    int ch, ix, iy;
+    long long p = dC.split(idx, ch);
+    p = dW.split(p, ix); int n = (int)dH.split(p, iy);
+    int oy = iy >> 1, ox = ix >> 1;
+    Chunk<T> o; o.raw = (u32x4){0u, 0u, 0u, 0u};
+    if (oy < Ho && ox < Wo) {
+      const size_t po = (((size_t)n * Ho + oy) * Wo + ox) * C + ch * CE;
+      Chunk<T> d, m;
+      d.raw = *(const u32x4*)(dy + po); m.raw = *(const u32x4*)(py + po);
+      unsigned cw[2] = {0u, 0u};
+      if constexpr (CE == 8) { const u32x2 c2 = *(const u32x2*)(code + po); cw[0] = c2[0]; cw[1] = c2[1]; }
+      else cw[0] = *(const unsigned*)(code + po);
+      const unsigned me = (unsigned)((iy & 1) * 2 + (ix & 1));
+      float ov[CE];
+#pragma unroll
+      for (int e = 0; e < CE; ++e) {
+        const unsigned am = (cw[e >> 2] >> (8 * (e & 3))) & 0xffu;
+        ov[e] = (am == me && m.get(e) > 0.f) ? d.get(e) : 0.f;
+      }
+      o.pack(ov);
+    }
+    *(u32x4*)(dx + (size_t)idx * CE) = o.raw;
+  }
+}
+extern "C" int s2p_maxpool2x2_bwd_idx(int dtype, const void* dy, const void* pool_y, const void* pool_idx, int N, int H, int W, int C,
+                                      void* dx, void* stream) {
+  S2P_REQUIRE(is_dtype(dtype), "s2p_maxpool2x2_bwd_idx: bad dtype");
+  S2P_REQUIRE(N >= 0 && H >= 0 && W >= 0 && C >= 0, "s2p_maxpool2x2_bwd_idx: negative size");
+  int Ho = H / 2, Wo = W / 2, ce = dtype == S2P_F32 ? 4 : 8;
+  if (C % ce) S2P_FAIL(-1, "s2p_maxpool2x2_bwd_idx: C must be a multiple of %d", ce);
+  long long total = (long long)N * H * W * (C / ce);
+  if (total == 0) return 0;
+  S2P_REQUIRE(dx && ((dy && pool_y && pool_idx) || (long long)Ho * Wo == 0), "s2p_maxpool2x2_bwd_idx: null pointer");
+  S2P_REQUIRE(host_al16(dy, pool_y, pool_idx, dx), "s2p_maxpool2x2_bwd_idx: dy, pool_y, pool_idx and dx must be 16-byte aligned");
+  if (dtype == S2P_F32) hipLaunchKernelGGL(maxpool_bwd_idx_kernel<float>, dim3(grid_for(total)), dim3(256), 0, (hipStream_t)stream, (const float*)dy, (const float*)pool_y, (const unsigned char*)pool_idx, N, H, W, C, (float*)dx, Ho, Wo);
+  else hipLaunchKernelGGL(maxpool_bwd_idx_kernel<__bf16>, dim3(grid_for(total)), dim3(256), 0, (hipStream_t)stream, (const __bf16*)dy, (const __bf16*)pool_y, (const unsigned char*)pool_idx, N, H, W, C, (__bf16*)dx, Ho, Wo);
+  S2P_CHECK_LAUNCH("maxpool_bwd_idx_kernel");
+  return 0;
 }
 extern "C" int s2p_maxpool2x2_fwd(int dtype, const void* x, int N, int H, int W, int C, void* y, void* stream) {
   S2P_REQUIRE(is_dtype(dtype), "s2p_maxpool2x2_fwd: bad dtype");
diff --git a/s2p_amd/csrc/s2p_common.h b/s2p_amd/csrc/s2p_common.h
--- a/s2p_amd/csrc/s2p_common.h
+++ b/s2p_amd/csrc/s2p_common.h
@@ -84,6 +84,27 @@
     }
   }
 };
+
+__device__ __forceinline__ void pool2x2_chunk(const Chunk<__bf16> (&v)[4], Chunk<__bf16>& o, u32x2& code) {
+  float ov[8];
+  unsigned c[2] = {0u, 0u};
+#pragma unroll
+  for (int e = 0; e < 8; ++e) {
+    ov[e] = fmaxf(fmaxf(v[0].get(e), v[1].get(e)), fmaxf(v[2].get(e), v[3].get(e)));
+    int a[4];
+#pragma unroll
+    for (int k = 0; k < 4; ++k) {
+      const unsigned w = v[k].raw[e >> 1];
+      const int s = (int)(short)((e & 1) ? (w >> 16) : (w & 0xffffu));
+      a[k] = s < 0 ? 0 : s;
+    }
+    const int m01 = a[0] > a[1] ? a[0] : a[1], m23 = a[2] > a[3] ? a[2] : a[3], m = m01 > m23 ? m01 : m23;
+    const unsigned am = a[0] == m ? 0u : (a[1] == m ? 1u : (a[2] == m ? 2u : 3u));
+    c[e >> 2] |= am << (8 * (e & 3));
+  }
+  o.pack(ov);
+  code = (u32x2){c[0], c[1]};
+}
 
 __device__ __forceinline__ double s2p_rcp_f64(int d) {
   const double x = (double)d;
diff --git a/s2p_amd/models/autograd_nodes.py b/s2p_amd/models/autograd_nodes.py
--- a/s2p_amd/models/autograd_nodes.py
+++ b/s2p_amd/models/autograd_nodes.py
@@ -88,7 +88,7 @@
     real_image.record_stream(vs)
     with torch.cuda.stream(vs):
         real_nhwc = ops.nchw_to_nhwc(real_image, dt, ce)
-        taps, acts = model.vgg.fwd_nhwc(real_nhwc)
+        taps, acts = model.vgg.fwd_nhwc(real_nhwc, need_bwd=False)
     return dict(real_nhwc=real_nhwc, taps=taps, acts=acts, stream=vs)
 
 
@@ -161,7 +161,7 @@
                 if pre is not None:
                     taps_r, vctx_real = pre["taps"], pre["acts"]
                 else:
-                    taps_r, vctx_real = model.vgg.fwd_nhwc(real_nhwc)
+                    taps_r, vctx_real = model.vgg.fwd_nhwc(real_nhwc, need_bwd=False)
                 taps, vctx = model.vgg.fwd_nhwc(fake)
                 tap_grads = [torch.empty_like(t) for t in taps]
                 ops.l1_loss_multi([(t, tr, opt.lambda_vgg * wk / t.numel(), losses[2:3], tg)
diff --git a/s2p_amd/models/networks/layers.py b/s2p_amd/models/networks/layers.py
--- a/s2p_amd/models/networks/layers.py
+++ b/s2p_amd/models/networks/layers.py
@@ -19,6 +19,10 @@
     def fwd(self, x, act=ACT_NONE, slope=0.2, aux=None, epi=EPI_STORE, y_pitch=None):
         return ops.conv_fwd(self.geom, x, self.pk.w_fwd, self.pk.bias, self.cin_pad(x.dtype), y_pitch=y_pitch,
                             act=act, slope=slope, aux=aux, epi=epi)
+
+    def fwd_pool(self, x, act=ACT_RELU, want_y=False, want_idx=True):
+        return ops.conv_fwd_pool(self.geom, x, self.pk.w_fwd, self.pk.bias, self.cin_pad(x.dtype), act=act, want_y=want_y,
+                                 want_idx=want_idx)
 
     def _group_major(self, t5):
         g = self.geom
diff --git a/s2p_amd/models/networks/loss.py b/s2p_amd/models/networks/loss.py
--- a/s2p_amd/models/networks/loss.py
+++ b/s2p_amd/models/networks/loss.py
@@ -17,6 +17,18 @@
 VGG_WEIGHTS = (1.0 / 32, 1.0 / 16, 1.0 / 8, 1.0 / 4, 1.0)
 TORCHVISION_IDX = dict(conv1_1=0, conv1_2=2, conv2_1=5, conv2_2=7, conv3_1=10, conv3_2=12, conv3_3=14, conv3_4=16,
                        conv4_1=19, conv4_2=21, conv4_3=23, conv4_4=25, conv5_1=28)
+
+
+FUSE_POOL = True
+
+
+class PrePool:
+
+    def __init__(self, lay, xin, shape, pool_y, pool_idx):
+        self.lay, self.xin, self.shape, self.pool_y, self.pool_idx = lay, xin, tuple(shape), pool_y, pool_idx
+
+    def detach(self):
+        return self.lay.fwd(self.xin, act=ACT_RELU)
 
 
 class VGG19(BaseNetwork):
@@ -63,18 +75,28 @@
             pk = self.store.pack(name, [m.weight], [m.bias], dtype=dt)
             self.lay[name] = ConvLayer(pk, ConvGeom(cin, cout, 3, 1, 1, net="VGG"))
 
-    def fwd_nhwc(self, x):
+    def fwd_nhwc(self, x, need_bwd=True):
         self._require_ready()
         acts = []
         h = x
         taps = []
-        for item in VGG_CFG:
+        for i, item in enumerate(VGG_CFG):
             if item == "P":
-                o = ops.maxpool_fwd(h)
+                if isinstance(h, PrePool):
+                    o = h.pool_y
+                else:
+                    o = ops.maxpool_fwd(h)
                 acts.append(("P", None, h, o))
             else:
                 name = item[0]
-                o = self.lay[name].fwd(h, act=ACT_RELU)
+                o = None
+                if FUSE_POOL and name not in VGG_TAPS and i + 1 < len(VGG_CFG) and VGG_CFG[i + 1] == "P":
+                    r = self.lay[name].fwd_pool(h, act=ACT_RELU, want_idx=need_bwd)
+                    if r is not None:
+                        N, H, W, _ = h.shape
+                        o = PrePool(self.lay[name], h, (N, H, W, r[1].shape[3]), r[1], r[2])
+                if o is None:
+                    o = self.lay[name].fwd(h, act=ACT_RELU)
                 acts.append(("C", name, h, o))
                 if name in VGG_TAPS:
                     taps.append(o)
@@ -85,12 +107,17 @@
         tapg = dict(zip(VGG_TAPS, tap_grads))
         d = None
         for kind, name, xin, out in reversed(acts):
-            xin_f, out_f = xin[:n_fake], out[:n_fake]
             if kind == "P":
-                d = ops.maxpool_bwd(d, xin_f)
+                if isinstance(xin, PrePool):
+                    if xin.pool_idx is None:
+                        raise RuntimeError("VGG19.bwd_nhwc: this forward was run with need_bwd=False")
+                    d = ops.maxpool_bwd_idx(d, xin.pool_y[:n_fake], xin.pool_idx[:n_fake], xin.shape[1], xin.shape[2])
+                else:
+                    d = ops.maxpool_bwd(d, xin[:n_fake])
                 continue
+            xin_f = xin[:n_fake]
             if d is None:
-                d = ops.act_bwd(tapg[name], out_f, ACT_RELU)
+                d = ops.act_bwd(tapg[name], out[:n_fake], ACT_RELU)
             lay = self.lay[name]
             if name == "conv1_1":
                 return lay.dgrad(d, xin_f.shape)
diff --git a/s2p_amd/ops.py b/s2p_amd/ops.py
--- a/s2p_amd/ops.py
+++ b/s2p_amd/ops.py
@@ -100,6 +100,30 @@
                                   ptr(ws), need, stream()), "s2p_conv2d_fwd")
     pr.done()
     return y
+
+
+_CAN_POOL = {}
+
+
+def conv_fwd_pool(geom, x, w_fwd, bias, cin_pad, act=ACT_RELU, want_y=False, want_idx=True):
+    N, H, W, xp = x.shape
+    Ho, Wo = geom.out_hw(H, W)
+    y_pitch = pad_to(geom.cout, chunk_elems(x.dtype))
+    d = geom.desc(x.dtype, N, H, W, cin_pad, xp, y_pitch)
+    key = (geom.cin, geom.cout, geom.k, geom.stride, geom.pad, geom.transposed, geom.reflect, geom.groups, geom.output_padding,
+           x.dtype, N, H, W, cin_pad, xp, act)
+    if key not in _CAN_POOL:
+        _CAN_POOL[key] = bool(lib().s2p_conv2d_fwd_can_pool(ctypes.byref(d), act))
+    if not _CAN_POOL[key]:
+        return None
+    y = torch.empty((N, Ho, Wo, y_pitch), dtype=x.dtype, device=x.device) if want_y else None
+    pool_y = torch.empty((N, Ho // 2, Wo // 2, y_pitch), dtype=x.dtype, device=x.device)
+    pool_idx = torch.empty((N, Ho // 2, Wo // 2, y_pitch), dtype=torch.uint8, device=x.device) if want_idx else None
+    pr = _Prof("fwd", geom, N, H, W, x.dtype)
+    check(lib().s2p_conv2d_fwd_pool(ctypes.byref(d), ptr(x), ptr(w_fwd), ptr(bias), ptr(y), ptr(pool_y), ptr(pool_idx), act,
+                                    stream()), "s2p_conv2d_fwd_pool")
+    pr.done()
+    return y, pool_y, pool_idx
 
 
 def conv_fwd_mat(geom, x, w_fwd, bias, cin_pad, gb, gb_off, gb_st, st_off, act=ACT_LRELU, slope=0.2, aux=None, epi=EPI_STORE,
@@ -373,6 +397,14 @@
     return dx
 
 
+def maxpool_bwd_idx(dy, pool_y, pool_idx, H, W):
+    N, _, _, C = pool_y.shape
+    dx = torch.empty((N, H, W, C), dtype=pool_y.dtype, device=pool_y.device)
+    check(lib().s2p_maxpool2x2_bwd_idx(dtype_id(pool_y.dtype), ptr(dy), ptr(pool_y), ptr(pool_idx), N, H, W, C, ptr(dx),
+                                       stream()), "s2p_maxpool2x2_bwd_idx")
+    return dx
+
+
 def resize_nearest(x, Ho, Wo):
     N, H, W, C = x.shape
     y = torch.empty((N, Ho, Wo, C), dtype=x.dtype, device=x.device)
```

Measured after the change: 8173 images/sec, median of 6. +1.1%, better.
